# crate-crypto/rust-eth-kzg

Measured on AMD Instinct MI355X. Metric: blobs/sec compute_cells_and_kzg_proofs (4096-pt blob), higher is better.
Workload: dtype u32

## Files before the change

### rust-eth-kzg_amd/csrc/engine.hip

```cpp
#include "engine_internal.hpp"

namespace kzg {

static Fr fr_from_u64(uint64_t v) {
    Fr a = zero<FrParams>();
    a.v[0] = (uint32_t)v;
    a.v[1] = (uint32_t)(v >> 32);
    return to_mont(a);
}
static Fr fr_pow_limbs(const Fr& base, const uint32_t* e, int nl) {
    Fr acc = one<FrParams>();
    for (int i = 32 * nl - 1; i >= 0; i--) {
        acc = sqr(acc);
        if ((e[i >> 5] >> (i & 31)) & 1) acc = mul(acc, base);
    }
    return acc;
}
static Fr fr_root_of_unity(int log_n) {
    uint32_t e[8];
    for (int i = 0; i < 8; i++) e[i] = FrParams::MOD[i];
    e[0] -= 1;
    for (int s = 0; s < log_n; s++) {
        for (int i = 0; i < 8; i++) e[i] = (e[i] >> 1) | (i < 7 ? (e[i + 1] << 31) : 0);
    }
    return fr_pow_limbs(fr_from_u64(7), e, 8);
}
typedef unsigned __int128 u128;
static const u128 GLV_LAMBDA = ((u128)0xac45a4010001a402ULL << 64) | 0x00000000ffffffffULL;
static void glv_split(const Fr& canon, u128& k1, u128& k2) {
    u128 rem = 0, q = 0;
    for (int i = 255; i >= 0; i--) {
        bool top = (rem >> 127) & 1;
        rem = (rem << 1) | ((canon.v[i >> 5] >> (i & 31)) & 1);
        q <<= 1;
        if (top || rem >= GLV_LAMBDA) { rem -= GLV_LAMBDA; q |= 1; }
    }
    k1 = rem;
    k2 = q;
}
static void recode_glv_wnaf(const Fr& k_mont, const Fr& lambda_mont, uint32_t* out) {
    constexpr int TWW = launch::TWIDDLE_WORDS, W = launch::TWIDDLE_WNAF_W;
    u128 r, q;
    glv_split(from_mont(k_mont), r, q);
    struct Half { u128 mag; bool neg; };
    auto signed_sub = [](u128 a, u128 b) { return a >= b ? Half{a - b, false} : Half{b - a, true}; };
    const Half cand[4][2] = {
        {Half{r, false}, Half{q, false}},
        {signed_sub(r, GLV_LAMBDA), Half{q + 1, false}},
        {signed_sub(r, 1), signed_sub(q, GLV_LAMBDA + 1)},
        {signed_sub(r, GLV_LAMBDA + 1), signed_sub(q, GLV_LAMBDA)},
    };
    auto fr_of = [](const Half& h) {
        Fr a = zero<FrParams>();
        for (int i = 0; i < 4; i++) a.v[i] = (uint32_t)(h.mag >> (32 * i));
        a = to_mont(a);
        return h.neg ? neg(a) : a;
    };
    auto naf = [&](const Half& h, int8_t* dg, int& len, int& weight) {
        u128 v = h.mag;
        len = weight = 0;
        for (int t = 0; v != 0; t++, v >>= 1) {
            if (t >= 4 * TWW) throw std::runtime_error("constant recoding too long");
            if (!(v & 1)) continue;
            int d = (int)(v & ((1u << W) - 1));
            if (d >= (1 << (W - 1))) d -= 1 << W;
            if (d < 0) v += (u128)(-d); else v -= (u128)d;
            dg[t] = (int8_t)(h.neg ? -d : d);
            len = t + 1;
            weight++;
        }
    };
    double best_cost = 0;
    int best = -1;
    std::vector<uint32_t> best_words;
    for (int c = 0; c < 4; c++) {
        if (!eq(add(fr_of(cand[c][0]), mul(fr_of(cand[c][1]), lambda_mont)), k_mont)) throw std::runtime_error("GLV split failed");
        std::vector<uint32_t> words(2 * TWW, 0u);
        int len[2], wt[2];
        for (int h = 0; h < 2; h++) naf(cand[c][h], reinterpret_cast<int8_t*>(&words[(size_t)h * TWW]), len[h], wt[h]);
        const double cost = linmap::COST_DBL * std::max(len[0], len[1]) + 5.0e3 * (wt[0] + wt[1]);
        if (best < 0 || cost < best_cost) { best = c; best_cost = cost; best_words = words; }
    }
    for (int i = 0; i < 2 * TWW; i++) out[i] = best_words[i];
    for (int h = 0; h < 2; h++) {
        const int8_t* dg = reinterpret_cast<const int8_t*>(out + (size_t)h * TWW);
        Fr back = zero<FrParams>(), pw = one<FrParams>();
        for (int t = 0; t < 4 * TWW; t++, pw = add(pw, pw)) {
            const int d = dg[t];
            if (!d) continue;
            Fr term = pw;
            for (int m = 1; m < (d < 0 ? -d : d); m++) term = add(term, pw);
            back = d < 0 ? sub(back, term) : add(back, term);
        }
        if (!eq(back, fr_of(cand[best][h]))) throw std::runtime_error("constant recoding failed");
    }
}
double trace_clock_ms() {
    static const auto t0 = std::chrono::steady_clock::now();
    return std::chrono::duration<double, std::milli>(std::chrono::steady_clock::now() - t0).count();
}
static thread_local std::string t_last_error;
const std::string& Engine::last_error() const { return t_last_error; }
void Engine::set_error(const std::exception& e) { t_last_error = e.what(); }

BufferPool::~BufferPool() {
    for (auto& f : free_) {
        if (host_) (void)hipHostFree(f.second);
        else (void)hipFree(f.second);
    }
}
void* BufferPool::get(size_t bytes, size_t* cls) {
    size_t c = 256;
    while (c < bytes) c <<= 1;
    *cls = c;
    for (size_t i = 0; i < free_.size(); i++)
        if (free_[i].first == c) {
            void* p = free_[i].second;
            free_[i] = free_.back();
            free_.pop_back();
            pooled_ -= c;
            return p;
        }
    void* p = nullptr;
    hipError_t e = host_ ? hipHostMalloc(&p, c, hipHostMallocDefault) : hipMalloc(&p, c);
    if (e != hipSuccess) {
        (void)hipGetLastError();
        for (auto& f : free_) { if (host_) (void)hipHostFree(f.second); else (void)hipFree(f.second); }
        free_.clear();
        pooled_ = 0;
        e = host_ ? hipHostMalloc(&p, c, hipHostMallocDefault) : hipMalloc(&p, c);
        if (e != hipSuccess) throw std::runtime_error(host_ ? "hipHostMalloc failed" : "hipMalloc failed");
    }
    return p;
}
void BufferPool::put(void* p, size_t cls) {
    constexpr size_t KEEP = 6ull << 30;
    if (pooled_ + cls > KEEP) {
        if (host_) (void)hipHostFree(p); else (void)hipFree(p);
        return;
    }
    free_.emplace_back(cls, p);
    pooled_ += cls;
}
PoolBuf::PoolBuf(Engine& e, size_t bytes, bool pinned_host) : e_(e), host_(pinned_host) {
    p = (host_ ? e_.pin_pool_ : e_.dev_pool_).get(bytes ? bytes : 1, &cls_);
}
PoolBuf::~PoolBuf() {
    (void)hipStreamSynchronize(e_.stream_);
    (host_ ? e_.pin_pool_ : e_.dev_pool_).put(p, cls_);
}

std::atomic<bool> g_exiting{false};
std::mutex g_engines_mu;
std::vector<Engine*> g_engines;
void Engine::stop_builder() {
    cancel_build_.store(true);
    if (builder_.joinable()) builder_.join();
}
void stop_all_builders_at_exit() {
    g_exiting.store(true);
    std::vector<Engine*> live;
    {
        std::lock_guard<std::mutex> lk(g_engines_mu);
        live = g_engines;
    }
    for (Engine* e : live) e->stop_builder();
}

Engine::SerialLease Engine::lease_serial() {
    return lanes_.lease(this, max_lanes_, auxiliary_, [this] {
        try {
            return std::unique_ptr<Engine>(new Engine(use_precomp_, dev_, this));
        } catch (...) {
            (void)hipGetLastError();
            throw;
        }
    });
}

Engine::Engine(bool use_precomp, int device, const Engine* primary, double table_budget_gb) : dev_(device), use_precomp_(use_precomp), primary_(primary), auxiliary_(primary != nullptr) {
    knobs_ = primary ? primary->knobs_ : Knobs::from_env();
    if (knobs_.serial_lanes) max_lanes_ = knobs_.serial_lanes;
    if (knobs_.device_batch_max) device_batch_max_ = ((knobs_.device_batch_max + 63) / 64) * 64;
    if (use_precomp) {
        if (launch::glv_width_supported(knobs_.glv_window)) want_glv_c_ = knobs_.glv_window;
        if (table_budget_gb != 0) table_budget_gb_ = table_budget_gb;
        else if (knobs_.table_budget_gb != 0) table_budget_gb_ = knobs_.table_budget_gb;
    }
    vm_search_ = knobs_.vm_search;
    arena_signed_ = knobs_.arena_signed;
    msm_split_ = knobs_.msm_split;
    if (knobs_.pip_shift_min >= 1) pip_shift_min_ = knobs_.pip_shift_min;
#ifdef KZG_CIRC_MAX
    circ_max_ = KZG_CIRC_MAX;
#else
    circ_max_ = 2;
#endif
    try {
        construct();
    } catch (...) {
        teardown();
        throw;
    }
}

void Engine::construct() {
    const bool trace = knobs_.trace;
    auto t0 = std::chrono::steady_clock::now();
    auto lap = [&](const char* what) {
        if (!trace) return;
        auto t1 = std::chrono::steady_clock::now();
        fprintf(stderr, "[context] %-28s %8.1f ms\n", what, std::chrono::duration<double, std::milli>(t1 - t0).count());
        t0 = t1;
    };
    HIPCK(hipSetDevice(dev_));
    {
        int cus = 0;
        HIPCK(hipDeviceGetAttribute(&cus, hipDeviceAttributeMultiprocessorCount, dev_));
        wave_slots_ = cus * 4 * 2;
        if (knobs_.msm_chunks >= 0) msm_chunks_ = knobs_.msm_chunks;
    }
    HIPCK(hipStreamCreateWithFlags(&stream_, hipStreamNonBlocking));
    if (!primary_) {
        int prio_low = 0, prio_high = 0;
        HIPCK(hipDeviceGetStreamPriorityRange(&prio_low, &prio_high));
        HIPCK(hipStreamCreateWithPriority(&build_stream_, hipStreamNonBlocking, prio_low));
    }
    if (v_two_streams_) HIPCK(hipStreamCreateWithFlags(&v_side_, hipStreamNonBlocking));
    HIPCK(hipEventCreateWithFlags(&v_decoded_, hipEventDisableTiming));
    HIPCK(hipEventCreateWithFlags(&v_checked_, hipEventDisableTiming));
    for (Work& w : work_) {
        HIPCK(hipEventCreateWithFlags(&w.done, hipEventDisableTiming));
        HIPCK(hipEventCreateWithFlags(&w.ev_in, hipEventDisableTiming));
        HIPCK(hipEventCreateWithFlags(&w.ev_cells, hipEventDisableTiming));
        HIPCK(hipEventCreateWithFlags(&w.ev_cells_host, hipEventDisableTiming));
        HIPCK(hipEventCreateWithFlags(&w.ev_done, hipEventDisableTiming));
        HIPCK(hipEventCreateWithFlags(&w.ev_coeffs, hipEventDisableTiming));
        HIPCK(hipEventCreateWithFlags(&w.ev_side, hipEventDisableTiming));
        if (&w == &work_[0]) continue;
        if (primary_) continue;
        int prio_low = 0, prio_high = 0;
        HIPCK(hipDeviceGetStreamPriorityRange(&prio_low, &prio_high));
        HIPCK(hipStreamCreateWithFlags(&w.stream, hipStreamNonBlocking));
        HIPCK(hipStreamCreateWithPriority(&w.copy, hipStreamNonBlocking, prio_high));
    }
    launch::init_attributes();
    if (!primary_) settle_streams();
    lap("HIP runtime + stream");
    init_constants();
    lap("twiddles, recodings");
    init_srs();
    lap("SRS decompress");
    init_fk20();
    lap("FK20 bases + start tables");
    init_verifier();
    HIPCK(hipStreamSynchronize(stream_));
    lap("verifier (G2 lines, cosets)");
    if (knobs_.fault == "constructor" && !primary_) throw std::runtime_error("injected fault (ETH_KZG_AMD_FAULT=constructor)");
    start_builder();
}

bool Engine::streams_overlap(hipStream_t a, hipStream_t b) {
    int khz = 0;
    if (hipDeviceGetAttribute(&khz, hipDeviceAttributeWallClockRate, dev_) != hipSuccess || khz <= 0) khz = 100000;
    const double spin_us = 300.0;
    const uint64_t ticks = (uint64_t)(spin_us * 1e-3 * khz);
    for (int t = 0; t < 3; t++) {
        HIPCK(hipStreamSynchronize(a));
        HIPCK(hipStreamSynchronize(b));
        const auto t0 = std::chrono::steady_clock::now();
        launch::spin(ticks, a);
        launch::spin(ticks, b);
        HIPCK(hipStreamSynchronize(a));
        HIPCK(hipStreamSynchronize(b));
        const double us = std::chrono::duration<double, std::micro>(std::chrono::steady_clock::now() - t0).count();
        if (us < 1.6 * spin_us) return true;
    }
    return false;
}
void Engine::settle_streams() {
    const bool trace = knobs_.trace;
    launch::spin(1, stream_);
    std::vector<hipStream_t> chosen{stream_}, rejected;
    bool gave_up = false;
    for (int i = 1; i < NW; i++) {
        Work& w = work_[i];
        if (!w.stream || gave_up) continue;
        for (int attempt = 0;; attempt++) {
            launch::spin(1, w.stream);
            bool ok = true;
            for (hipStream_t c : chosen) ok = ok && streams_overlap(c, w.stream);
            if (ok || attempt == 5) {
                if (trace) fprintf(stderr, "[eth_kzg_amd] work set %d: stream %s after %d replacement(s)\n", i, ok ? "runs beside the others" : "still shares a queue", attempt);
                if (!ok) gave_up = true;
                break;
            }
            rejected.push_back(w.stream);
            HIPCK(hipStreamCreateWithFlags(&w.stream, hipStreamNonBlocking));
        }
        chosen.push_back(w.stream);
    }
    for (hipStream_t r : rejected) hipStreamDestroy(r);
}

Engine::~Engine() { teardown(); }

void Engine::teardown() noexcept {
    (void)hipSetDevice(dev_);
    lanes_.clear();
    stop_builder();
    {
        std::lock_guard<std::mutex> lk(g_engines_mu);
        g_engines.erase(std::remove(g_engines.begin(), g_engines.end(), this), g_engines.end());
    }
    if (build_stream_) hipStreamDestroy(build_stream_);
    host_pool_.reset();
    vm_pool_.reset();
    stage_pool_.reset();
    void* ptrs[] = {d_w8192_, d_w29_, d_naf_, d_srs_, d_fk_bases_, d_in_, d_cells_, d_proofs_, d_coset_, d_coset_inv_, d_circ_terms_};
    for (void* p : ptrs)
        if (p) hipFree(p);
    for (SlpProgram& P : slp_prog_) {
        if (P.d_words) hipFree(P.d_words);
        if (P.d_naf && P.owns_naf) hipFree(P.d_naf);
    }
    for (Work& w : work_) {
        void* dev[] = {w.coeffs, w.canon, w.scalars, w.X, w.status, w.circ_table, w.slp_arena, w.d_in, w.d_cells, w.d_proofs};
        for (void* p : dev)
            if (p) hipFree(p);
        void* pin[] = {w.h_in, w.h_cells, w.h_proofs, w.h_status};
        for (void* p : pin)
            if (p) hipHostFree(p);
        hipEvent_t evs[] = {w.done, w.ev_in, w.ev_cells, w.ev_cells_host, w.ev_done, w.ev_coeffs, w.ev_side};
        for (hipEvent_t e : evs)
            if (e) hipEventDestroy(e);
        for (hipEvent_t e : w.sub_events) hipEventDestroy(e);
        if (w.stream) hipStreamDestroy(w.stream);
        if (w.copy) hipStreamDestroy(w.copy);
    }
    if (v_dev_) hipFree(v_dev_);
    if (v_pin_) hipHostFree(v_pin_);
    for (VmSlot& v : vm_slot_) {
        if (v.dev) hipFree(v.dev);
        if (v.pin) hipHostFree(v.pin);
        if (v.vs.dev) hipFree(v.vs.dev);
        if (v.vs.pin) hipHostFree(v.vs.pin);
    }
    if (vd_pin_) hipHostFree(vd_pin_);
    for (hipEvent_t e : vd_events_)
        if (e) hipEventDestroy(e);
    if (v_side_) hipStreamDestroy(v_side_);
    if (v_decoded_) hipEventDestroy(v_decoded_);
    if (v_checked_) hipEventDestroy(v_checked_);
    if (stream_) hipStreamDestroy(stream_);
}

void Engine::init_constants() {
    std::vector<Fr> w(N_EXT);
    Fr g = fr_root_of_unity(13);
    w[0] = one<FrParams>();
    for (int i = 1; i < N_EXT; i++) w[i] = mul(w[i - 1], g);
    if (!eq(mul(w[N_EXT - 1], g), one<FrParams>())) throw std::runtime_error("omega_8192 has wrong order");
    HIPCK(hipMalloc(&d_w8192_, N_EXT * sizeof(Fr)));
    HIPCK(hipMemcpy(d_w8192_, w.data(), N_EXT * sizeof(Fr), hipMemcpyHostToDevice));
    {
        std::vector<uint32_t> w29((size_t)N_EXT * 9);
        launch::ntt_twiddles29(w.data(), w29.data());
        HIPCK(hipMalloc(&d_w29_, w29.size() * 4));
        HIPCK(hipMemcpy(d_w29_, w29.data(), w29.size() * 4, hipMemcpyHostToDevice));
    }
    {
        Fr lam = zero<FrParams>();
        for (int i = 0; i < 4; i++) lam.v[i] = (uint32_t)(GLV_LAMBDA >> (32 * i));
        Fr lm = to_mont(lam);
        if (!is_zero(add(add(sqr(lm), lm), one<FrParams>()))) throw std::runtime_error("GLV lambda is not a cube root of unity");
        constexpr int TWW = launch::TWIDDLE_WORDS;
        std::vector<uint32_t> tw((size_t)128 * 2 * TWW, 0u);
        for (int k = 0; k < 128; k++) recode_glv_wnaf(w[64 * k], lm, &tw[(size_t)k * 2 * TWW]);
        HIPCK(hipMalloc(&d_naf_, tw.size() * 4));
        HIPCK(hipMemcpy(d_naf_, tw.data(), tw.size() * 4, hipMemcpyHostToDevice));
        std::vector<uint32_t> plus, minus;
        int max_t = 0;
        for (int d = 0; d < 128; d++) {
            Fr c = zero<FrParams>();
            for (int t = 0; t < 64; t++) c = add(c, w[(64 * d * t) & (N_EXT - 1)]);
            if (d != 0 && (d & 1) == 0) {
                if (!is_zero(c)) throw std::runtime_error("circulant symbol: even entry is not zero");
                continue;
            }
            u128 kk[2];
            glv_split(from_mont(c), kk[0], kk[1]);
            Fr back = zero<FrParams>();
            for (int half = 0; half < 2; half++) {
                u128 k = kk[half];
                Fr pw = half ? lm : one<FrParams>();
                for (int t = 0; k != 0; t++, k >>= 1, pw = add(pw, pw)) {
                    if (!(k & 1)) continue;
                    const int dg = 2 - (int)(k & 3);
                    if (dg < 0) k += 1;
                    const uint32_t word = (uint32_t)d | ((uint32_t)t << 7) | ((uint32_t)half << 15) | ((dg < 0 ? 1u : 0u) << 16) | (1u << 17);
                    (dg < 0 ? minus : plus).push_back(word);
                    back = dg < 0 ? sub(back, pw) : add(back, pw);
                    if (t > max_t) max_t = t;
                }
            }
            if (!eq(back, c)) throw std::runtime_error("circulant term list does not reproduce its symbol");
        }
        if ((int)plus.size() < launch::CIRC_LANES || max_t >= 255) throw std::runtime_error("circulant term list is malformed");
        std::vector<uint32_t> all(plus);
        all.insert(all.end(), minus.begin(), minus.end());
        circ_T_ = max_t + 1;
        circ_per_lane_ = ((int)all.size() + launch::CIRC_LANES - 1) / launch::CIRC_LANES;
        all.resize((size_t)circ_per_lane_ * launch::CIRC_LANES, 0u);
        HIPCK(hipMalloc(&d_circ_terms_, all.size() * 4));
        HIPCK(hipMemcpy(d_circ_terms_, all.data(), all.size() * 4, hipMemcpyHostToDevice));
    }
    init_linmap(reinterpret_cast<const Fr8*>(w.data()));
    for (int sgi = 0; sgi < 3; sgi++) {
        Fr v = zero<FrParams>();
        v.v[sgi + 1] = 1;
        v = to_mont(v);
        memcpy(&seg_shift_[sgi], &v, 32);
    }
    Fr i4096 = inv(fr_from_u64(N_BLOB)), i128 = inv(fr_from_u64(128));
    memcpy(&n_inv4096_, &i4096, 32);
    memcpy(&inv128_, &i128, 32);
}

static linmap::Strategy slp_strategy(int id) {
    linmap::Strategy s;
    s.allow_toom8 = true;
    auto fixed = [&](int k4, int k8, int k16, int k32) {
        s.tuned = false;
        s.balanced_lincomb = true;
        s.hankel_split = {{2, 2}, {4, k4}, {8, k8}, {16, k16}, {32, k32}};
    };
    switch (id) {
        case 2: fixed(2, 2, 2, 2); break;
        case 3: fixed(4, 2, 4, 2); break;
        case 4: fixed(2, 2, 2, 4); break;
        case 5: fixed(4, 2, 4, 8); break;
        default: break;
    }
    return s;
}
void Engine::build_slp_program(int id) {
    const Fr* w128p = reinterpret_cast<const Fr*>(w128_.data());
    const std::vector<Fr> w128(w128p, w128p + 128);
    const bool verbose = knobs_.trace;
    linmap::Plan plan = linmap::build_fk20_proofs_plan(w128, slp_strategy(id), verbose);
    {
        std::vector<linmap::Ref> perm(128);
        for (int p = 0; p < 128; p++) {
            int k = 0;
            for (int b = 0; b < 7; b++) k |= ((p >> b) & 1) << (6 - b);
            perm[p] = plan.outputs[k];
        }
        plan.outputs = perm;
    }
    const linmap::Schedule sched = linmap::make_schedule(plan, id == SLP_TUNED_FUSED);
    uint64_t st = 0x853c49e6748fea9bull + (uint64_t)id;
    for (int it = 0; it < 2; it++) {
        std::vector<Fr> in(128);
        for (auto& v : in) {
            for (int i = 0; i < 8; i++) { st ^= st << 13; st ^= st >> 7; st ^= st << 17; v.v[i] = (uint32_t)(st >> 16); }
            v.v[7] &= 0x3fffffffu;
        }
        const auto want = linmap::fk20_proofs_map_by_definition(w128, in);
        const auto got1 = linmap::run_over_fr(plan, in);
        const auto got2 = linmap::run_schedule_over_fr(sched, plan.consts, 128, 128, in);
        for (int p = 0; p < 128; p++) {
            int k = 0;
            for (int b = 0; b < 7; b++) k |= ((p >> b) & 1) << (6 - b);
            if (!eq(want[k], got1[p]) || !eq(want[k], got2[p])) throw std::runtime_error("FK20 proofs map: compiled program differs from its definition");
        }
    }
    SlpProgram& P = slp_prog_[id];
    if (id == SLP_TUNED && slp_prog_[SLP_TUNED_FUSED].ready) {
        P.d_naf = slp_prog_[SLP_TUNED_FUSED].d_naf;
    } else {
        Fr lam = zero<FrParams>();
        for (int i = 0; i < 4; i++) lam.v[i] = (uint32_t)(GLV_LAMBDA >> (32 * i));
        const Fr lm = to_mont(lam);
        constexpr int TWW = launch::TWIDDLE_WORDS;
        std::vector<uint32_t> naf(plan.consts.size() * 2 * TWW);
        for (size_t c = 0; c < plan.consts.size(); c++) recode_glv_wnaf(plan.consts[c], lm, &naf[c * 2 * TWW]);
        HIPCK(hipMalloc(&P.d_naf, naf.size() * 4));
        P.owns_naf = true;
        HIPCK(hipMemcpy(P.d_naf, naf.data(), naf.size() * 4, hipMemcpyHostToDevice));
    }
    HIPCK(hipMalloc(&P.d_words, sched.words.size() * 4));
    HIPCK(hipMemcpy(P.d_words, sched.words.data(), sched.words.size() * 4, hipMemcpyHostToDevice));
    P.launches.clear();
    for (auto& L : sched.launches) P.launches.push_back(SlpLaunch{(int)L.kind, L.first, L.count});
    P.n_slots = sched.n_slots;
    P.info[0] = (int)plan.count(linmap::OP_MULC);
    P.info[1] = (int)(plan.count(linmap::OP_ADD) + plan.count(linmap::OP_SUB));
    P.info[2] = (int)plan.doublings();
    P.info[3] = (int)sched.launches.size();
    if (verbose) fprintf(stderr, "[linmap] program %d: %d multiplications, %d additions, %d doublings, %d launches, %d slots\n", id, P.info[0], P.info[1], P.info[2], P.info[3], P.n_slots);
    P.ready = true;
}
const Engine::SlpProgram& Engine::slp_program(int id) {
    std::lock_guard<std::mutex> lk(slp_build_mu_);
    if (!slp_prog_[id].ready) build_slp_program(id);
    return slp_prog_[id];
}
int Engine::pick_slp_program(int lanes) const {
    if (slp_force_ >= 0) return slp_force_;
    const int groups = lanes / 64, simds = wave_slots_ / 2;
    if (712 * groups <= simds) return SLP_KARATSUBA;
    if (456 * groups <= simds) return SLP_DEPTH_456;
    if (606 * groups <= wave_slots_) return SLP_DEPTH_606;
    if (456 * groups <= wave_slots_) return SLP_DEPTH_456;
    if (372 * groups <= wave_slots_) return SLP_DEPTH_372;
    if (456 * groups <= wave_slots_ * 3 / 2) return SLP_DEPTH_456;
    if (groups <= 12) return SLP_DEPTH_372;
    return lanes >= slp_fuse_min_ ? SLP_TUNED_FUSED : SLP_TUNED;
}
void Engine::init_linmap(const Fr8* w8192_mont) {
    static_assert(sizeof(Fr8) == sizeof(Fr), "layout");
    if (knobs_.slp_program >= 0 && knobs_.slp_program < SLP_COUNT) slp_force_ = knobs_.slp_program;
    w128_.resize(128);
    for (int e = 0; e < 128; e++) w128_[e] = w8192_mont[64 * e];
    build_slp_program(SLP_TUNED_FUSED);
    build_slp_program(SLP_TUNED);
    const SlpProgram& fused = slp_prog_[SLP_TUNED_FUSED];
    {
        if (fused.info[0] != slp_prog_[SLP_TUNED].info[0]) throw std::runtime_error("FK20 proofs map: the two schedules differ");
    }
    for (int i = 0; i < 3; i++) slp_info_[i] = fused.info[i];
    slp_info_[3] = fused.info[3];
    const Fr h = inv(fr_from_u64(2));
    memcpy(&half_, &h, 32);
}

void Engine::init_srs() {
    const unsigned char* p = kzg_srs_begin;
    size_t len = (size_t)(kzg_srs_end - kzg_srs_begin);
    uint32_t n1, n2;
    if (len < 16 || memcmp(p, "KZGSRS01", 8)) throw std::runtime_error("bad embedded SRS");
    memcpy(&n1, p + 8, 4);
    memcpy(&n2, p + 12, 4);
    if (n1 != (uint32_t)N_BLOB || len != 16 + (size_t)n1 * 48 + (size_t)n2 * 96) throw std::runtime_error("bad embedded SRS size");
    uint8_t* d_bytes;
    int* d_st;
    HIPCK(hipMalloc(&d_bytes, (size_t)N_BLOB * 48));
    HIPCK(hipMalloc(&d_st, N_BLOB * sizeof(int)));
    HIPCK(hipMalloc(&d_srs_, N_BLOB * sizeof(G1Affine)));
    HIPCK(hipMemcpy(d_bytes, p + 16, (size_t)N_BLOB * 48, hipMemcpyHostToDevice));
    {
        Fp12w nobeta{};
        launch::g1_decompress(d_bytes, d_srs_, d_st, N_BLOB, 0, nobeta, stream_);
    }
    std::vector<int> st(N_BLOB);
    HIPCK(hipMemcpyAsync(st.data(), d_st, N_BLOB * sizeof(int), hipMemcpyDeviceToHost, stream_));
    HIPCK(hipStreamSynchronize(stream_));
    for (int s : st)
        if (s) throw std::runtime_error("embedded SRS point failed to decompress");
    HIPCK(hipFree(d_bytes));
    HIPCK(hipFree(d_st));
    {
        G1Affine P;
        HIPCK(hipMemcpy(&P, (const G1Affine*)d_srs_ + 1, sizeof(G1Affine), hipMemcpyDeviceToHost));
        uint32_t lam[4];
        for (int i = 0; i < 4; i++) lam[i] = (uint32_t)(GLV_LAMBDA >> (32 * i));
        G1Affine Q = to_affine(scalar_mul<4>(to_jac(P), lam));
        Fp bx = mul(Q.x, inv(P.x));
        Fp b3 = mul(sqr(bx), bx);
        if (!eq(b3, one<FpParams>()) || eq(bx, one<FpParams>()) || !eq(Q.y, P.y)) throw std::runtime_error("GLV endomorphism check failed");
        memcpy(&beta_, &bx, 48);
    }
}

}
```

### rust-eth-kzg_amd/csrc/g1_linmap.hpp

```cpp
#pragma once
#include "field.hpp"

#include <algorithm>
#include <cstdint>
#include <cstdio>
#include <functional>
#include <map>
#include <stdexcept>
#include <tuple>
#include <vector>

namespace kzg {
namespace linmap {

enum OpKind : uint8_t { OP_ADD = 0, OP_SUB = 1, OP_DBL = 2, OP_MULC = 3 };
struct Op {
    OpKind kind;
    int dst;
    int a;
    int b;
};
struct Ref {
    int id = -1;
    bool neg = false;
    bool zero() const { return id < 0; }
};

struct Plan {
    int n_in = 0;
    int n_values = 0;
    std::vector<Op> ops;
    std::vector<Ref> outputs;
    std::vector<Fr> consts;
    long count(OpKind k) const {
        long n = 0;
        for (auto& o : ops) n += o.kind == k;
        return n;
    }
    long doublings() const {
        long n = 0;
        for (auto& o : ops) n += o.kind == OP_DBL ? o.b : 0;
        return n;
    }
};

constexpr double COST_MULC = 690e3, COST_ADD = 8.3e3, COST_DBL = 3.1e3;

inline Fr fr_small(int64_t v) {
    Fr a = zero<FrParams>();
    uint64_t m = v < 0 ? (uint64_t)(-v) : (uint64_t)v;
    a.v[0] = (uint32_t)m;
    a.v[1] = (uint32_t)(m >> 32);
    a = to_mont(a);
    return v < 0 ? neg(a) : a;
}

class Builder {
public:
    explicit Builder(int n_in) {
        plan_.n_in = n_in;
        plan_.n_values = n_in;
    }
    Ref input(int i) const { return Ref{i, false}; }
    static Ref negate(Ref r) { return r.zero() ? r : Ref{r.id, !r.neg}; }

    Ref add(Ref a, Ref b) {
        if (a.zero()) return b;
        if (b.zero()) return a;
        if (a.id == b.id) return a.neg == b.neg ? dbl(a, 1) : Ref{};
        if (!a.neg && !b.neg) return Ref{emit2(OP_ADD, a.id, b.id, true), false};
        if (a.neg && b.neg) return Ref{emit2(OP_ADD, a.id, b.id, true), true};
        if (!a.neg) return Ref{emit2(OP_SUB, a.id, b.id, false), false};
        return Ref{emit2(OP_SUB, b.id, a.id, false), false};
    }
    Ref sub(Ref a, Ref b) { return add(a, negate(b)); }
    Ref dbl(Ref a, int t) {
        if (a.zero() || t == 0) return a;
        auto key = std::make_tuple((int)OP_DBL, a.id, t);
        auto it = memo_.find(key);
        if (it != memo_.end()) return Ref{it->second, a.neg};
        int id = plan_.n_values++;
        plan_.ops.push_back(Op{OP_DBL, id, a.id, t});
        memo_[key] = id;
        return Ref{id, a.neg};
    }
    Ref mulc(Ref a, const Fr& c) {
        if (a.zero() || is_zero(c)) return Ref{};
        if (eq(c, one<FrParams>())) return a;
        if (eq(c, neg(one<FrParams>()))) return negate(a);
        int cid = (int)plan_.consts.size();
        plan_.consts.push_back(c);
        int id = plan_.n_values++;
        plan_.ops.push_back(Op{OP_MULC, id, a.id, cid});
        return Ref{id, a.neg};
    }
    Ref lincomb(const std::vector<std::pair<Ref, int64_t>>& terms) {
        std::vector<std::pair<Ref, uint64_t>> t;
        int top = -1;
        for (auto& pr : terms) {
            if (pr.first.zero() || pr.second == 0) continue;
            Ref r = pr.second < 0 ? negate(pr.first) : pr.first;
            uint64_t m = pr.second < 0 ? (uint64_t)(-pr.second) : (uint64_t)pr.second;
            t.emplace_back(r, m);
            for (int b = 63; b >= 0; b--)
                if ((m >> b) & 1) { if (b > top) top = b; break; }
        }
        Ref acc;
        int pending = 0;
        for (int b = top; b >= 0; b--) {
            if (!acc.zero()) pending++;
            if (b == top) pending = 0;
            for (auto& pr : t)
                if ((pr.second >> b) & 1) {
                    if (pending) { acc = dbl(acc, pending); pending = 0; }
                    acc = add(acc, pr.first);
                }
        }
        if (pending) acc = dbl(acc, pending);
        return acc;
    }
    Ref lincomb_balanced(const std::vector<std::pair<Ref, int64_t>>& terms) {
        struct T { Ref r; int e; };
        std::vector<T> t;
        for (auto& pr : terms) {
            if (pr.first.zero() || pr.second == 0) continue;
            const uint64_t m = pr.second < 0 ? (uint64_t)(-pr.second) : (uint64_t)pr.second;
            if (m & (m - 1)) return lincomb(terms);
            int e = 0;
            while (!((m >> e) & 1)) e++;
            t.push_back(T{pr.second < 0 ? negate(pr.first) : pr.first, e});
        }
        if (t.empty()) return Ref{};
        std::stable_sort(t.begin(), t.end(), [](const T& a, const T& b) { return a.e < b.e; });
        std::function<Ref(int, int)> rec = [&](int lo, int hi) -> Ref {
            if (hi - lo == 1) return t[lo].r;
            const int mid = (lo + hi) / 2;
            const Ref a = rec(lo, mid), b = rec(mid, hi);
            return add(dbl(b, t[mid].e - t[lo].e), a);
        };
        return dbl(rec(0, (int)t.size()), t[0].e);
    }
    Plan take(const std::vector<Ref>& outputs) {
        plan_.outputs = outputs;
        return std::move(plan_);
    }
    const Plan& plan() const { return plan_; }
    double cost() const { return plan_.count(OP_MULC) * COST_MULC + (plan_.count(OP_ADD) + plan_.count(OP_SUB)) * COST_ADD + plan_.doublings() * COST_DBL; }

private:
    int emit2(OpKind k, int a, int b, bool commutative) {
        if (commutative && a > b) std::swap(a, b);
        auto key = std::make_tuple((int)k, a, b);
        auto it = memo_.find(key);
        if (it != memo_.end()) return it->second;
        int id = plan_.n_values++;
        plan_.ops.push_back(Op{k, id, a, b});
        memo_[key] = id;
        return id;
    }
    Plan plan_;
    std::map<std::tuple<int, int, int>, int> memo_;
};

struct EvalPoint { int a, b; };
inline std::vector<EvalPoint> toom_points(int k) {
    switch (k) {
        case 2: return {{0, 1}, {1, 0}, {1, 1}};
        case 3: return {{0, 1}, {1, 0}, {1, 1}, {-1, 1}, {2, 1}};
        case 4: return {{0, 1}, {1, 0}, {1, 1}, {-1, 1}, {2, 1}, {-2, 1}, {1, 2}};
        case 8: return {{0, 1}, {1, 0}, {1, 1}, {-1, 1}, {2, 1}, {-2, 1}, {1, 2}, {-1, 2}, {4, 1}, {-4, 1}, {1, 4}, {-1, 4}, {8, 1}, {-8, 1}, {1, 8}};
        default: throw std::runtime_error("toom_points: unsupported split");
    }
}
inline int64_t ipow(int64_t b, int e) {
    int64_t r = 1;
    while (e-- > 0) r *= b;
    return r;
}
inline std::vector<std::vector<Fr>> toom_fixed_side(int k) {
    const auto pts = toom_points(k);
    const int R = 2 * k - 1;
    std::vector<std::vector<Fr>> M(R, std::vector<Fr>(2 * R, zero<FrParams>()));
    for (int s = 0; s < R; s++) {
        for (int r = 0; r < R; r++) M[s][r] = fr_small(ipow(pts[r].a, s) * ipow(pts[r].b, 2 * k - 2 - s));
        M[s][R + s] = one<FrParams>();
    }
    for (int col = 0; col < R; col++) {
        int piv = -1;
        for (int row = col; row < R; row++)
            if (!is_zero(M[row][col])) { piv = row; break; }
        if (piv < 0) throw std::runtime_error("toom: singular evaluation matrix");
        std::swap(M[piv], M[col]);
        const Fr iv = inv(M[col][col]);
        for (int j = 0; j < 2 * R; j++) M[col][j] = mul(M[col][j], iv);
        for (int row = 0; row < R; row++) {
            if (row == col || is_zero(M[row][col])) continue;
            const Fr f = M[row][col];
            for (int j = 0; j < 2 * R; j++) M[row][j] = sub(M[row][j], mul(f, M[col][j]));
        }
    }
    std::vector<std::vector<Fr>> U(R, std::vector<Fr>(R));
    for (int r = 0; r < R; r++)
        for (int D = 0; D < R; D++) U[r][D] = M[r][R + D];
    return U;
}

class Compiler {
public:
    std::map<int, int> hankel_split;
    std::map<int, bool> root_split;
    bool allow_toom8 = true;
    bool balanced_lincomb = false;
    Ref sum(Builder& B, const std::vector<std::pair<Ref, int64_t>>& t) const { return balanced_lincomb ? B.lincomb_balanced(t) : B.lincomb(t); }

    std::vector<Ref> hankel(Builder& B, const std::vector<Ref>& x, const std::vector<Fr>& h) {
        const int n = (int)x.size();
        if ((int)h.size() != 2 * n - 1) throw std::runtime_error("hankel: size mismatch");
        if (n == 1) return {B.mulc(x[0], h[0])};
        const int k = hankel_split.count(n) ? hankel_split[n] : 2;
        if (n % k) throw std::runtime_error("hankel: split does not divide the size");
        const int m = n / k, R = 2 * k - 1;
        const auto pts = toom_points(k);
        const auto& U = fixed_side(k);
        std::vector<std::vector<Ref>> X(R, std::vector<Ref>(m));
        std::vector<int> partner(R, -1);
        for (int r = 0; r < R; r++)
            for (int q = 0; q < R; q++)
                if (q != r && pts[q].a == -pts[r].a && pts[q].b == pts[r].b && pts[r].a > 0) { partner[r] = q; partner[q] = r; }
        for (int r = 0; r < R; r++) {
            if (partner[r] >= 0 && pts[r].a < 0) continue;
            for (int i = 0; i < m; i++) {
                if (partner[r] < 0) {
                    std::vector<std::pair<Ref, int64_t>> t;
                    for (int J = 0; J < k; J++) t.emplace_back(x[J * m + i], ipow(pts[r].a, J) * ipow(pts[r].b, k - 1 - J));
                    X[r][i] = sum(B, t);
                } else {
                    std::vector<std::pair<Ref, int64_t>> ev, od;
                    for (int J = 0; J < k; J++) (J & 1 ? od : ev).emplace_back(x[J * m + i], ipow(pts[r].a, J) * ipow(pts[r].b, k - 1 - J));
                    const Ref e = sum(B, ev), o = sum(B, od);
                    X[r][i] = B.add(e, o);
                    X[partner[r]][i] = B.sub(e, o);
                }
            }
        }
        std::vector<std::vector<Ref>> Z(R);
        for (int r = 0; r < R; r++) {
            std::vector<Fr> hr(2 * m - 1, zero<FrParams>());
            for (int D = 0; D < R; D++) {
                if (is_zero(U[r][D])) continue;
                for (int s = 0; s < 2 * m - 1; s++) hr[s] = add(hr[s], mul(U[r][D], h[D * m + s]));
            }
            Z[r] = hankel(B, X[r], hr);
        }
        std::vector<Ref> y(n);
        for (int i = 0; i < m; i++) {
            std::vector<Ref> S(R), Dm(R);
            for (int r = 0; r < R; r++)
                if (partner[r] >= 0 && pts[r].a > 0) {
                    S[r] = B.add(Z[r][i], Z[partner[r]][i]);
                    Dm[r] = B.sub(Z[r][i], Z[partner[r]][i]);
                }
            for (int I = 0; I < k; I++) {
                std::vector<std::pair<Ref, int64_t>> t;
                for (int r = 0; r < R; r++) {
                    if (partner[r] >= 0 && pts[r].a < 0) continue;
                    const int64_t coef = ipow(pts[r].a, I) * ipow(pts[r].b, k - 1 - I);
                    if (partner[r] < 0) t.emplace_back(Z[r][i], coef);
                    else t.emplace_back((I & 1) ? Dm[r] : S[r], coef);
                }
                y[I * m + i] = sum(B, t);
            }
        }
        return y;
    }

    template <class SqrtFn>
    std::vector<Ref> twisted_cyclic(Builder& B, const std::vector<Ref>& x, const std::vector<Fr>& c, const Fr& z, SqrtFn&& sqrt_of) {
        const int n = (int)x.size();
        Fr s;
        if (n >= 2 && root_split.count(n) && root_split[n] && sqrt_of(z, s)) {
            const int hn = n / 2;
            const Fr half = inv(fr_small(2)), s_inv = inv(s);
            std::vector<Ref> x1(hn), x2(hn);
            std::vector<Fr> c1(hn), c2(hn);
            for (int i = 0; i < hn; i++) {
                const Ref t = B.mulc(x[hn + i], s);
                x1[i] = B.add(x[i], t);
                x2[i] = B.sub(x[i], t);
                const Fr sc = mul(s, c[hn + i]);
                c1[i] = mul(half, add(c[i], sc));
                c2[i] = mul(half, sub(c[i], sc));
            }
            const auto y1 = twisted_cyclic(B, x1, c1, s, sqrt_of);
            const auto y2 = twisted_cyclic(B, x2, c2, neg(s), sqrt_of);
            std::vector<Ref> y(n);
            for (int i = 0; i < hn; i++) {
                y[i] = B.add(y1[i], y2[i]);
                y[hn + i] = B.mulc(B.sub(y1[i], y2[i]), s_inv);
            }
            return y;
        }
        std::vector<Fr> h(2 * n - 1);
        for (int u = 0; u < 2 * n - 1; u++) {
            const int d = u - (n - 1);
            h[u] = d >= 0 ? c[d] : mul(z, c[n + d]);
        }
        std::vector<Ref> xr(n);
        for (int j = 0; j < n; j++) xr[j] = x[n - 1 - j];
        return hankel(B, xr, h);
    }

    template <class SqrtFn>
    std::vector<Ref> cyclic(Builder& B, const std::vector<Ref>& x, const std::vector<Fr>& c, SqrtFn&& sqrt_of) {
        const int n = (int)x.size();
        if (n == 1) return {B.mulc(x[0], c[0])};
        const int hn = n / 2;
        const Fr half = inv(fr_small(2));
        std::vector<Ref> xp(hn), xm(hn);
        std::vector<Fr> cp(hn), cm(hn);
        for (int i = 0; i < hn; i++) {
            xp[i] = B.add(x[i], x[hn + i]);
            xm[i] = B.sub(x[i], x[hn + i]);
            cp[i] = mul(half, add(c[i], c[hn + i]));
            cm[i] = mul(half, sub(c[i], c[hn + i]));
        }
        const auto yp = cyclic(B, xp, cp, sqrt_of);
        const auto ym = twisted_cyclic(B, xm, cm, neg(one<FrParams>()), sqrt_of);
        std::vector<Ref> y(n);
        for (int i = 0; i < hn; i++) {
            y[i] = B.add(yp[i], ym[i]);
            y[hn + i] = B.sub(yp[i], ym[i]);
        }
        return y;
    }

    void tune(int max_n) {
        uint64_t st = 0x9e3779b97f4a7c15ull;
        auto rnd_fr = [&]() {
            Fr a;
            for (int i = 0; i < 8; i++) { st ^= st << 13; st ^= st >> 7; st ^= st << 17; a.v[i] = (uint32_t)(st >> 16); }
            a.v[7] &= 0x3fffffffu;
            return a;
        };
        auto no_sqrt = [](const Fr&, Fr&) { return false; };
        auto any_sqrt = [&](const Fr&, Fr& s) { s = rnd_fr(); return true; };
        for (int n = 2; n <= max_n; n *= 2) {
            double best = 0;
            int best_k = 0;
            for (int k : {2, 4, 8}) {
                if (n % k || (k == 8 && !allow_toom8)) continue;
                hankel_split[n] = k;
                Builder B(n);
                std::vector<Ref> x(n);
                for (int i = 0; i < n; i++) x[i] = B.input(i);
                std::vector<Fr> h(2 * n - 1);
                for (auto& v : h) v = rnd_fr();
                hankel(B, x, h);
                if (!best_k || B.cost() < best) { best = B.cost(); best_k = k; }
            }
            hankel_split[n] = best_k;
            double cost[2];
            for (int split = 0; split < 2; split++) {
                root_split[n] = split != 0;
                Builder B(n);
                std::vector<Ref> x(n);
                for (int i = 0; i < n; i++) x[i] = B.input(i);
                std::vector<Fr> c(n);
                for (auto& v : c) v = rnd_fr();
                if (split) twisted_cyclic(B, x, c, rnd_fr(), any_sqrt);
                else twisted_cyclic(B, x, c, rnd_fr(), no_sqrt);
                cost[split] = B.cost();
            }
            root_split[n] = cost[1] < cost[0];
        }
    }

private:
    const std::vector<std::vector<Fr>>& fixed_side(int k) {
        auto it = fixed_.find(k);
        if (it == fixed_.end()) it = fixed_.emplace(k, toom_fixed_side(k)).first;
        return it->second;
    }
    std::map<int, std::vector<std::vector<Fr>>> fixed_;
};

inline std::vector<Fr> run_over_fr(const Plan& p, const std::vector<Fr>& in) {
    std::vector<Fr> v(p.n_values, zero<FrParams>());
    for (int i = 0; i < p.n_in; i++) v[i] = in[i];
    for (auto& o : p.ops) {
        switch (o.kind) {
            case OP_ADD: v[o.dst] = add(v[o.a], v[o.b]); break;
            case OP_SUB: v[o.dst] = sub(v[o.a], v[o.b]); break;
            case OP_DBL: { Fr t = v[o.a]; for (int k = 0; k < o.b; k++) t = add(t, t); v[o.dst] = t; break; }
            case OP_MULC: v[o.dst] = mul(v[o.a], p.consts[o.b]); break;
        }
    }
    std::vector<Fr> out(p.outputs.size());
    for (size_t i = 0; i < out.size(); i++) {
        const Ref r = p.outputs[i];
        out[i] = r.zero() ? zero<FrParams>() : (r.neg ? neg(v[r.id]) : v[r.id]);
    }
    return out;
}

struct Strategy {
    bool tuned = true, allow_toom8 = true;
    std::map<int, int> hankel_split;
    std::map<int, bool> root_split;
    bool balanced_lincomb = false;
};
inline Plan build_fk20_proofs_plan(const std::vector<Fr>& w128, const Strategy& strat, bool verbose = false) {
    if (w128.size() != 128) throw std::runtime_error("w128: need the 128 powers");
    auto sqrt_of = [&](const Fr& z, Fr& s) {
        for (int e = 0; e < 128; e += 2)
            if (eq(z, w128[e])) { s = w128[e / 2]; return true; }
        return false;
    };
    Compiler C;
    C.allow_toom8 = strat.allow_toom8;
    C.balanced_lincomb = strat.balanced_lincomb;
    if (strat.tuned) C.tune(32);
    else { C.hankel_split = strat.hankel_split; C.root_split = strat.root_split; }
    Builder B(128);
    const Fr one_ = one<FrParams>(), inv32 = inv(fr_small(32));
    auto m_of = [&](int e) {
        return mul(inv32, inv(sub(one_, w128[((e % 128) + 128) % 128])));
    };
    std::vector<Ref> even(64), odd(64);
    for (int a = 0; a < 64; a++) { even[a] = B.input(2 * a); odd[a] = B.input(2 * a + 1); }
    std::vector<Fr> c1(64), c2(64);
    for (int d = 0; d < 64; d++) { c1[d] = m_of(2 * d - 1); c2[d] = m_of(2 * d + 1); }
    const auto t1 = C.cyclic(B, odd, c1, sqrt_of);
    const auto t2 = C.cyclic(B, even, c2, sqrt_of);
    std::vector<Ref> out(128);
    for (int a = 0; a < 64; a++) {
        out[2 * a] = B.add(even[a], t1[a]);
        out[2 * a + 1] = B.add(odd[a], t2[a]);
    }
    for (auto& r : out)
        if (r.zero() || r.neg || r.id < 128) throw std::runtime_error("fk20 plan: degenerate output");
    Plan p = B.take(out);
    if (verbose) {
        fprintf(stderr, "[linmap] hankel splits:");
        for (auto& kv : C.hankel_split) fprintf(stderr, " %d->%d", kv.first, kv.second);
        fprintf(stderr, "  root splits:");
        for (auto& kv : C.root_split) fprintf(stderr, " %d:%d", kv.first, (int)kv.second);
        fprintf(stderr, "\n[linmap] %ld constant multiplications, %ld additions, %ld doublings\n", p.count(OP_MULC),
                p.count(OP_ADD) + p.count(OP_SUB), p.doublings());
    }
    return p;
}
inline Plan build_fk20_proofs_plan(const std::vector<Fr>& w128, bool allow_toom8 = true, bool verbose = false) {
    Strategy s;
    s.allow_toom8 = allow_toom8;
    return build_fk20_proofs_plan(w128, s, verbose);
}

inline std::vector<Fr> fk20_proofs_map_by_definition(const std::vector<Fr>& w128, const std::vector<Fr>& in) {
    const Fr inv64 = inv(fr_small(64));
    std::vector<Fr> h(64), out(128);
    for (int n = 0; n < 64; n++) {
        Fr acc = zero<FrParams>();
        for (int j = 0; j < 128; j++) acc = add(acc, mul(in[j], w128[(128 - (j * n) % 128) % 128]));
        h[n] = mul(acc, inv64);
    }
    for (int k = 0; k < 128; k++) {
        Fr acc = zero<FrParams>();
        for (int n = 0; n < 64; n++) acc = add(acc, mul(h[n], w128[(k * n) % 128]));
        out[k] = acc;
    }
    return out;
}

struct Launch {
    OpKind kind;
    int first, count;
};
struct Schedule {
    int n_slots = 0;
    std::vector<uint32_t> words;
    std::vector<Launch> launches;
    long mulc_total = 0;
    long fused_pairs = 0;
    long fused_runs = 0;
};
inline Schedule make_schedule(const Plan& p, bool fuse_add_sub = true, bool fuse_runs = true) {
    const int n_out = (int)p.outputs.size();
    std::vector<char> live(p.n_values, 0);
    for (auto& r : p.outputs) live[r.id] = 1;
    for (int i = (int)p.ops.size() - 1; i >= 0; i--) {
        const Op& o = p.ops[i];
        if (!live[o.dst]) continue;
        live[o.a] = 1;
        if (o.kind == OP_ADD || o.kind == OP_SUB) live[o.b] = 1;
    }
    std::vector<int> run_of(p.n_values, 0);
    std::vector<int> run_src(p.n_values, -1);
    if (fuse_runs) {
        std::vector<std::vector<int>> users(p.n_values);
        std::vector<char> is_output(p.n_values, 0);
        for (auto& r : p.outputs) is_output[r.id] = 1;
        for (int i = 0; i < (int)p.ops.size(); i++) {
            const Op& o = p.ops[i];
            if (!live[o.dst]) continue;
            users[o.a].push_back(i);
            if (o.kind == OP_ADD || o.kind == OP_SUB) users[o.b].push_back(i);
        }
        for (auto& o : p.ops) {
            if (!live[o.dst] || o.kind != OP_DBL || is_output[o.dst] || o.b > 31) continue;
            const auto& u = users[o.dst];
            auto two = [&](int k) { return p.ops[k].kind == OP_ADD || p.ops[k].kind == OP_SUB; };
            auto fits = [&](const Op& c) {
                const int other = c.a == o.dst ? c.b : c.a;
                return c.a != c.b && !run_of[other] && (c.kind == OP_ADD || c.a == o.dst);
            };
            bool ok = false;
            if (u.size() == 1 && two(u[0]) && fits(p.ops[u[0]])) ok = true;
            if (fuse_add_sub && u.size() == 2 && two(u[0]) && two(u[1]) && p.ops[u[0]].kind != p.ops[u[1]].kind) {
                const Op &x = p.ops[u[0]], &y = p.ops[u[1]];
                if (std::min(x.a, x.b) == std::min(y.a, y.b) && std::max(x.a, x.b) == std::max(y.a, y.b) && fits(x) && fits(y)) ok = true;
            }
            if (!ok) continue;
            run_of[o.dst] = o.b;
            run_src[o.dst] = o.a;
        }
    }
    auto eff = [&](int v) { return run_of[v] ? run_src[v] : v; };
    std::vector<int> md(p.n_values, 0), lvl(p.n_values, 0);
    int max_md = 0;
    std::vector<int> max_lvl;
    for (auto& o : p.ops) {
        if (!live[o.dst]) continue;
        const bool two = o.kind == OP_ADD || o.kind == OP_SUB;
        if (run_of[o.dst]) {
            md[o.dst] = md[o.a];
            lvl[o.dst] = lvl[o.a];
            continue;
        }
        if (o.kind == OP_MULC) {
            md[o.dst] = md[o.a] + 1;
            lvl[o.dst] = 0;
        } else {
            md[o.dst] = two ? std::max(md[o.a], md[o.b]) : md[o.a];
            int l = 0;
            if (md[o.a] == md[o.dst]) l = std::max(l, lvl[o.a] + 1);
            if (two && md[o.b] == md[o.dst]) l = std::max(l, lvl[o.b] + 1);
            lvl[o.dst] = std::max(l, 1);
        }
        max_md = std::max(max_md, md[o.dst]);
        if ((int)max_lvl.size() <= md[o.dst]) max_lvl.resize(md[o.dst] + 1, 0);
        max_lvl[md[o.dst]] = std::max(max_lvl[md[o.dst]], lvl[o.dst]);
    }
    std::vector<std::vector<int>> step_ops;
    std::map<std::pair<int, int>, int> step_of;
    for (int ph = 0; ph <= max_md; ph++)
        for (int l = 0; l <= (ph < (int)max_lvl.size() ? max_lvl[ph] : 0); l++) {
            step_of[{ph, l}] = (int)step_ops.size();
            step_ops.emplace_back();
        }
    std::vector<int> def_step(p.n_values, -1), last_use(p.n_values, -1);
    for (int i = 0; i < (int)p.ops.size(); i++) {
        const Op& o = p.ops[i];
        if (!live[o.dst] || run_of[o.dst]) continue;
        const int s = step_of[{md[o.dst], lvl[o.dst]}];
        step_ops[s].push_back(i);
        def_step[o.dst] = s;
        last_use[eff(o.a)] = std::max(last_use[eff(o.a)], s);
        if (o.kind == OP_ADD || o.kind == OP_SUB) last_use[eff(o.b)] = std::max(last_use[eff(o.b)], s);
    }
    Schedule S;
    std::vector<int> slot(p.n_values, -1);
    for (int i = 0; i < p.n_in; i++) slot[i] = i;
    for (int k = 0; k < n_out; k++) {
        if (slot[p.outputs[k].id] >= 0) throw std::runtime_error("schedule: an output value is shared or is an input");
        slot[p.outputs[k].id] = p.n_in + k;
    }
    int next_slot = p.n_in + n_out;
    std::vector<int> free_list;
    std::vector<std::vector<int>> expire(step_ops.size() + 1);
    for (int v = p.n_in; v < p.n_values; v++)
        if (live[v] && slot[v] < 0 && last_use[v] >= 0) expire[last_use[v]].push_back(v);
    for (int s = 0; s < (int)step_ops.size(); s++) {
        for (int i : step_ops[s]) {
            const int v = p.ops[i].dst;
            if (slot[v] >= 0) continue;
            if (!free_list.empty()) { slot[v] = free_list.back(); free_list.pop_back(); }
            else slot[v] = next_slot++;
        }
        for (int v : expire[s]) free_list.push_back(slot[v]);
        std::map<std::pair<int, int>, int> add_of;
        for (int i : step_ops[s])
            if (p.ops[i].kind == OP_ADD) add_of[{std::min(p.ops[i].a, p.ops[i].b), std::max(p.ops[i].a, p.ops[i].b)}] = i;
        std::map<int, int> partner;
        std::vector<char> fused_away(p.ops.size(), 0);
        if (fuse_add_sub)
            for (int i : step_ops[s]) {
                if (p.ops[i].kind != OP_SUB) continue;
                auto it = add_of.find({std::min(p.ops[i].a, p.ops[i].b), std::max(p.ops[i].a, p.ops[i].b)});
                if (it == add_of.end() || fused_away[it->second]) continue;
                partner[i] = it->second;
                fused_away[it->second] = 1;
            }
        std::vector<int> ordered = step_ops[s];
        auto op_cost = [&](int i) {
            const Op& o = p.ops[i];
            if (o.kind == OP_DBL) return o.b * COST_DBL;
            if (o.kind == OP_MULC) return COST_MULC;
            return (run_of[o.a] + run_of[o.b]) * COST_DBL + (partner.count(i) ? 1.15 * COST_ADD : COST_ADD);
        };
        std::stable_sort(ordered.begin(), ordered.end(), [&](int x, int y) { return op_cost(x) > op_cost(y); });
        for (int pass = 0; pass < 2; pass++) {
            Launch L{pass == 0 ? OP_MULC : OP_ADD, (int)S.words.size() / 4, 0};
            for (int i : ordered) {
                const Op& o = p.ops[i];
                const bool two = o.kind == OP_ADD || o.kind == OP_SUB;
                if ((pass == 0) != (o.kind == OP_MULC)) continue;
                if (fused_away[i]) continue;
                int first = o.a, second = two ? o.b : 0;
                if (two && run_of[o.b]) std::swap(first, second);
                const uint32_t shifts = two ? (uint32_t)run_of[first] << 3 : 0u;
                if (two && run_of[first]) S.fused_runs++;
                if (partner.count(i)) {
                    S.words.push_back((uint32_t)slot[p.ops[partner[i]].dst]);
                    S.words.push_back((uint32_t)slot[eff(first)]);
                    S.words.push_back((uint32_t)slot[eff(second)]);
                    S.words.push_back(4u | shifts | ((uint32_t)slot[o.dst] << 16));
                    L.count++;
                    S.fused_pairs++;
                    continue;
                }
                S.words.push_back((uint32_t)slot[o.dst]);
                S.words.push_back((uint32_t)slot[two ? eff(first) : o.a]);
                S.words.push_back(two ? (uint32_t)slot[eff(second)] : (uint32_t)o.b);
                S.words.push_back((o.kind == OP_SUB ? 1u : o.kind == OP_DBL ? 2u : 0u) | shifts);
                L.count++;
            }
            if (L.count) S.launches.push_back(L);
            if (pass == 0) S.mulc_total += L.count;
        }
    }
    S.n_slots = next_slot;
    return S;
}

inline std::vector<Fr> run_schedule_over_fr(const Schedule& S, const std::vector<Fr>& consts, int n_in, int n_out, const std::vector<Fr>& in) {
    std::vector<Fr> arena(S.n_slots, zero<FrParams>());
    for (int i = 0; i < n_in; i++) arena[i] = in[i];
    for (auto& L : S.launches) {
        std::vector<Fr> res(L.count), res2(L.count);
        for (int i = 0; i < L.count; i++) {
            const uint32_t* w = &S.words[(size_t)(L.first + i) * 4];
            const Fr a = arena[w[1]];
            if (L.kind == OP_MULC) res[i] = mul(a, consts[w[2]]);
            else if (w[3] & 2u) { Fr t = a; for (uint32_t k = 0; k < w[2]; k++) t = add(t, t); res[i] = t; }
            else {
                Fr x = a, y = arena[w[2]];
                for (uint32_t k = 0; k < ((w[3] >> 3) & 31u); k++) x = add(x, x);
                if (w[3] & 4u) { res[i] = add(x, y); res2[i] = sub(x, y); }
                else res[i] = (w[3] & 1u) ? sub(x, y) : add(x, y);
            }
        }
        for (int i = 0; i < L.count; i++) {
            const uint32_t* w = &S.words[(size_t)(L.first + i) * 4];
            arena[w[0]] = res[i];
            if (L.kind != OP_MULC && (w[3] & 4u)) arena[w[3] >> 16] = res2[i];
        }
    }
    return std::vector<Fr>(arena.begin() + n_in, arena.begin() + n_in + n_out);
}

}
}
```

### rust-eth-kzg_amd/csrc/k_g1slp.hip

```cpp
#include "engine.hpp"
#include <stdexcept>
#include "g1_mulc.hpp"
#include "g1_mulc30.hpp"
#include "g1_coop.hpp"

namespace kzg {

static_assert(sizeof(JacS) == launch::SIZEOF_JACS && sizeof(JacQ) == launch::SIZEOF_JACQ, "the engine sizes and offsets the arena with these");

__global__ __launch_bounds__(64, 2) void k_slp_mulc(JacQ* __restrict__ A, int stride, const uint32_t* __restrict__ words,
                                                    const uint32_t* __restrict__ naf, Fs<1, DC> beta, int n_active) {
    const uint32_t* w = words + (size_t)blockIdx.x * 4;
    const uint32_t dst = __builtin_amdgcn_readfirstlane(w[0]), a = __builtin_amdgcn_readfirstlane(w[1]),
                   cid = __builtin_amdgcn_readfirstlane(w[2]);
    const int lane = (gridDim.y - 1 - blockIdx.y) * 64 + threadIdx.x;
    if (lane >= n_active) return;
    const JacQ src = A[(size_t)a * stride + lane];
    A[(size_t)dst * stride + lane] = mul_by_recoded30(src, naf + (size_t)cid * (2 * launch::TWIDDLE_WORDS), beta);
}
__global__ __launch_bounds__(64, 2) void k_slp_mulc_s(JacS* __restrict__ A, int stride, const uint32_t* __restrict__ words,
                                                      const uint32_t* __restrict__ naf, Fs<1, DC> beta, int n_active) {
    const uint32_t* w = words + (size_t)blockIdx.x * 4;
    const uint32_t dst = __builtin_amdgcn_readfirstlane(w[0]), a = __builtin_amdgcn_readfirstlane(w[1]),
                   cid = __builtin_amdgcn_readfirstlane(w[2]);
    const int lane = (gridDim.y - 1 - blockIdx.y) * 64 + threadIdx.x;
    const JacS src = A[(size_t)a * stride + (lane < n_active ? lane : n_active - 1)];
    const JacS r = mul_by_recoded30(src, naf + (size_t)cid * (2 * launch::TWIDDLE_WORDS), beta);
    if (lane < n_active) A[(size_t)dst * stride + lane] = r;
}
__global__ __launch_bounds__(64, 2) void k_slp_mulc_coop(JacQ* __restrict__ A, int stride, const uint32_t* __restrict__ words,
                                                         const uint32_t* __restrict__ naf, Fq<1> beta, int lanes) {
    const uint32_t* w = words + (size_t)blockIdx.x * 4;
    const uint32_t dst = __builtin_amdgcn_readfirstlane(w[0]), a = __builtin_amdgcn_readfirstlane(w[1]),
                   cid = __builtin_amdgcn_readfirstlane(w[2]);
    const int lane = blockIdx.y * 16 + (threadIdx.x >> 2), quad = threadIdx.x & 3;
    if (lane >= lanes) return;
    const JacQ src = A[(size_t)a * stride + lane];
    A[(size_t)dst * stride + lane] = mul_by_recoded<4>(src, naf + (size_t)cid * (2 * launch::TWIDDLE_WORDS), beta, quad);
}
__global__ __launch_bounds__(64, 2) void k_slp_mulc_coop2(JacQ* __restrict__ A, int stride, const uint32_t* __restrict__ words,
                                                          const uint32_t* __restrict__ naf, Fq<1> beta, int lanes) {
    const uint32_t* w = words + (size_t)blockIdx.x * 4;
    const uint32_t dst = __builtin_amdgcn_readfirstlane(w[0]), a = __builtin_amdgcn_readfirstlane(w[1]),
                   cid = __builtin_amdgcn_readfirstlane(w[2]);
    const int lane = blockIdx.y * 32 + (threadIdx.x >> 1), half = threadIdx.x & 1;
    if (lane >= lanes) return;
    const JacQ src = A[(size_t)a * stride + lane];
    A[(size_t)dst * stride + lane] = mul_by_recoded<2>(src, naf + (size_t)cid * (2 * launch::TWIDDLE_WORDS), beta, half);
}
__device__ __forceinline__ void slp_cheap_op(JacQ* __restrict__ A, int stride, int lane, uint32_t dst, uint32_t a, uint32_t b, uint32_t fl) {
    JacQ r = A[(size_t)a * stride + lane];
    const uint32_t runs = (fl & 2u) ? b : (fl >> 3) & 31u;
#pragma unroll 1
    for (uint32_t k = 0; k < runs; k++) r = dbl(r);
    bool degenerate = false;
    if (!(fl & 2u)) {
        if (fl & 4u) {
            const AddSubShared sh = add_sub_prepare(r, A[(size_t)b * stride + lane]);
            degenerate = sh.degenerate;
            A[(size_t)(fl >> 16) * stride + lane] = add_sub_finish(sh, true);
            r = add_sub_finish(sh, false);
        } else {
            r = add(r, A[(size_t)b * stride + lane], (fl & 1u) != 0);
        }
    }
    A[(size_t)dst * stride + lane] = r;
    if (degenerate) {
        asm volatile("" ::: "memory");
        JacQ p2 = A[(size_t)a * stride + lane];
#pragma unroll 1
        for (uint32_t k = 0; k < runs; k++) p2 = dbl(p2);
        const JacQ q2 = A[(size_t)b * stride + lane];
        const JacQ d = add_slow(p2, q2, true);
        A[(size_t)dst * stride + lane] = add_slow(p2, q2, false);
        A[(size_t)(fl >> 16) * stride + lane] = d;
    }
}
__global__ __launch_bounds__(64, 2) void k_slp_add(JacQ* __restrict__ A, int stride, const uint32_t* __restrict__ words, int n_active) {
    const uint32_t* w = words + (size_t)blockIdx.y * 4;
    const uint32_t dst = __builtin_amdgcn_readfirstlane(w[0]), a = __builtin_amdgcn_readfirstlane(w[1]),
                   b = __builtin_amdgcn_readfirstlane(w[2]), fl = __builtin_amdgcn_readfirstlane(w[3]);
    if ((int)(blockIdx.x * 64 + threadIdx.x) >= n_active) return;
    slp_cheap_op(A, stride, blockIdx.x * 64 + threadIdx.x, dst, a, b, fl);
}

__global__ __launch_bounds__(64, 2) void k_slp_add_s(JacS* __restrict__ A, int stride, const uint32_t* __restrict__ words, int n_active) {
    const uint32_t* w = words + (size_t)blockIdx.y * 4;
    const uint32_t dst = __builtin_amdgcn_readfirstlane(w[0]), a = __builtin_amdgcn_readfirstlane(w[1]),
                   b = __builtin_amdgcn_readfirstlane(w[2]), fl = __builtin_amdgcn_readfirstlane(w[3]);
    const int lane_of_thread = blockIdx.x * 64 + threadIdx.x;
    const bool keep = lane_of_thread < n_active;
    const int lane = keep ? lane_of_thread : n_active - 1;
    JacS r = A[(size_t)a * stride + lane];
    const uint32_t runs = (fl & 2u) ? b : (fl >> 3) & 31u;
#pragma unroll 1
    for (uint32_t k = 0; k < runs; k++) r = dbl_half(r);
    bool degenerate = false;
    if (!(fl & 2u)) {
        if (fl & 4u) {
            const AddSubSharedS sh = add_sub_prepare(r, A[(size_t)b * stride + lane]);
            degenerate = sh.degenerate;
            const JacS df = add_sub_finish(sh, true);
            if (keep) A[(size_t)(fl >> 16) * stride + lane] = df;
            r = add_sub_finish(sh, false);
        } else {
            r = add_unchecked(r, A[(size_t)b * stride + lane], (fl & 1u) != 0, degenerate);
        }
    }
    if (keep) A[(size_t)dst * stride + lane] = r;
    if (degenerate && keep) {
        asm volatile("" ::: "memory");
        JacS p2 = A[(size_t)a * stride + lane];
#pragma unroll 1
        for (uint32_t k = 0; k < runs; k++) p2 = dbl_half(p2);
        const JacS q2 = A[(size_t)b * stride + lane];
        if (fl & 4u) {
            const JacS d = add_slow(p2, q2, true);
            A[(size_t)dst * stride + lane] = add_slow(p2, q2, false);
            A[(size_t)(fl >> 16) * stride + lane] = d;
        } else {
            A[(size_t)dst * stride + lane] = add_slow(p2, q2, (fl & 1u) != 0);
        }
    }
}

__global__ __launch_bounds__(64, 2) void k_slp_add_coop(JacQ* __restrict__ A, int stride, const uint32_t* __restrict__ words, int lanes) {
    const uint32_t* w = words + (size_t)blockIdx.y * 4;
    const uint32_t dst = __builtin_amdgcn_readfirstlane(w[0]), a = __builtin_amdgcn_readfirstlane(w[1]),
                   b = __builtin_amdgcn_readfirstlane(w[2]), fl = __builtin_amdgcn_readfirstlane(w[3]);
    const int lane = blockIdx.x * 16 + (threadIdx.x >> 2), quad = threadIdx.x & 3;
    if (lane >= lanes) return;
    JacQ r = A[(size_t)a * stride + lane];
    const uint32_t runs = (fl & 2u) ? b : (fl >> 3) & 31u;
#pragma unroll 1
    for (uint32_t k = 0; k < runs; k++) r = coop_dbl(r, quad);
    if (!(fl & 2u)) {
        const JacQ q = A[(size_t)b * stride + lane];
        if (fl & 4u) {
            const JacQ d = coop_add(r, q, true, quad);
            A[(size_t)(fl >> 16) * stride + lane] = d;
            r = coop_add(r, q, false, quad);
        } else {
            r = coop_add(r, q, (fl & 1u) != 0, quad);
        }
    }
    A[(size_t)dst * stride + lane] = r;
}

template <int COOP>
__global__ __launch_bounds__(64, 2) void k_slp_mulc_coop_s(JacS* __restrict__ A, int stride, const uint32_t* __restrict__ words,
                                                           const uint32_t* __restrict__ naf, Fs<1, DC> beta, int lanes) {
    const uint32_t* w = words + (size_t)blockIdx.x * 4;
    const uint32_t dst = __builtin_amdgcn_readfirstlane(w[0]), a = __builtin_amdgcn_readfirstlane(w[1]),
                   cid = __builtin_amdgcn_readfirstlane(w[2]);
    const int lane_of_thread = blockIdx.y * (64 / COOP) + (threadIdx.x / COOP), sub = threadIdx.x % COOP;
    const bool keep = lane_of_thread < lanes;
    const int lane = keep ? lane_of_thread : lanes - 1;
    const JacS src = A[(size_t)a * stride + lane];
    const JacS r = mul_by_recoded30<COOP>(src, naf + (size_t)cid * (2 * launch::TWIDDLE_WORDS), beta, sub);
    if (keep) A[(size_t)dst * stride + lane] = r;
}
__global__ __launch_bounds__(64, 2) void k_slp_add_coop_s(JacS* __restrict__ A, int stride, const uint32_t* __restrict__ words, int lanes) {
    const uint32_t* w = words + (size_t)blockIdx.y * 4;
    const uint32_t dst = __builtin_amdgcn_readfirstlane(w[0]), a = __builtin_amdgcn_readfirstlane(w[1]),
                   b = __builtin_amdgcn_readfirstlane(w[2]), fl = __builtin_amdgcn_readfirstlane(w[3]);
    const int lane_of_thread = blockIdx.x * 16 + (threadIdx.x >> 2), quad = threadIdx.x & 3;
    const bool keep = lane_of_thread < lanes;
    const int lane = keep ? lane_of_thread : lanes - 1;
    JacS r = A[(size_t)a * stride + lane];
    const uint32_t runs = (fl & 2u) ? b : (fl >> 3) & 31u;
#pragma unroll 1
    for (uint32_t k = 0; k < runs; k++) r = coop4_dbl_half(r, quad);
    if (!(fl & 2u)) {
        const JacS q = A[(size_t)b * stride + lane];
        if (fl & 4u) {
            JacS d;
            coop4_add_sub(r, q, quad, r, d);
            if (keep) A[(size_t)(fl >> 16) * stride + lane] = d;
        } else {
            r = coop4_add(r, q, (fl & 1u) != 0, quad);
        }
    }
    if (keep) A[(size_t)dst * stride + lane] = r;
}

namespace launch {
void preload_k_g1slp() {
    hipFuncAttributes a;
    (void)hipFuncGetAttributes(&a, reinterpret_cast<const void*>(&k_slp_add));
}
void g1_slp_launch(int kind, void* arena, int stride, const uint32_t* words, int count, const void* naf, const Fp12w& beta,
                   hipStream_t st, int lanes, int coop_lanes, int fmt, int n_active) {
    if (lanes <= 0) lanes = stride;
    if (n_active <= 0 || n_active > lanes) n_active = lanes;
    const dim3 grid((unsigned)count, (unsigned)(lanes / 64));
    if (fmt == FMT_JACS) {
        const bool coop = coop_points_max() > 0;
        if (kind == 3) {
            Fp b384;
            for (int i = 0; i < 12; i++) b384.v[i] = beta.v[i];
            const Fs<1, DC> bs = fs_from_fp(b384);
            if (coop_lanes > 16 && coop)
                k_slp_mulc_coop_s<2><<<dim3((unsigned)count, (unsigned)((coop_lanes + 31) / 32)), 64, 0, st>>>((JacS*)arena, stride, words, (const uint32_t*)naf, bs, coop_lanes);
            else if (coop_lanes > 0 && coop)
                k_slp_mulc_coop_s<4><<<dim3((unsigned)count, (unsigned)((coop_lanes + 15) / 16)), 64, 0, st>>>((JacS*)arena, stride, words, (const uint32_t*)naf, bs, coop_lanes);
            else k_slp_mulc_s<<<grid, 64, 0, st>>>((JacS*)arena, stride, words, (const uint32_t*)naf, bs, n_active);
        } else {
            if (lanes == 64 && count * 4 <= 1024 && coop)
                k_slp_add_coop_s<<<dim3((unsigned)((n_active + 15) / 16), (unsigned)count), 64, 0, st>>>((JacS*)arena, stride, words, n_active);
            else k_slp_add_s<<<dim3((unsigned)(lanes / 64), (unsigned)count), 64, 0, st>>>((JacS*)arena, stride, words, n_active);
        }
        return;
    }
    if (kind == 3) {
        Fp b384;
        for (int i = 0; i < 12; i++) b384.v[i] = beta.v[i];
        if (coop_lanes > 16 && coop_points_max() > 0) {
            const dim3 g2((unsigned)count, (unsigned)((coop_lanes + 31) / 32));
            k_slp_mulc_coop2<<<g2, 64, 0, st>>>((JacQ*)arena, stride, words, (const uint32_t*)naf, fq_from_fp(b384), coop_lanes);
        }
        else if (coop_lanes > 0 && coop_points_max() > 0)
            k_slp_mulc_coop<<<dim3((unsigned)count, (unsigned)((coop_lanes + 15) / 16)), 64, 0, st>>>((JacQ*)arena, stride, words, (const uint32_t*)naf,
                                                                                                     fq_from_fp(b384), coop_lanes);
        else k_slp_mulc<<<grid, 64, 0, st>>>((JacQ*)arena, stride, words, (const uint32_t*)naf, fs_from_fp(b384), n_active);
    } else {
        if (lanes == 64 && count * 4 <= 1024 && coop_points_max() > 0)
            k_slp_add_coop<<<dim3((unsigned)((n_active + 15) / 16), (unsigned)count), 64, 0, st>>>((JacQ*)arena, stride, words, n_active);
        else k_slp_add<<<dim3((unsigned)(lanes / 64), (unsigned)count), 64, 0, st>>>((JacQ*)arena, stride, words, n_active);
    }
}
}
}
```

Before: 40230.

## Use GLV endomorphism rotations as free Toom evaluation points in G1 linear-map SLP

Extends the straight-line program builder so references can carry a cube-root-of-unity rotation, applied on the GPU as the cheap G1 endomorphism (x multiplied by beta). Toom-Cook Hankel splits may then use evaluation points times powers of lambda and ±1 (the mu6 class scheme), which allows larger splits such as 16 and fewer scalar-multiplication (MULC) ops in the FK20 proof linear map. The add kernels now take beta and rotate their operands according to flag bits, and the cost model constants are retuned. The risks are extra per-add field multiplications and more complex plans, and the fixed strategies turn phi off.

```diff
diff --git a/rust-eth-kzg_amd/csrc/engine.hip b/rust-eth-kzg_amd/csrc/engine.hip
--- a/rust-eth-kzg_amd/csrc/engine.hip
+++ b/rust-eth-kzg_amd/csrc/engine.hip
@@ -430,9 +430,15 @@
 static linmap::Strategy slp_strategy(int id) {
     linmap::Strategy s;
     s.allow_toom8 = true;
+    {
+        Fr lam = zero<FrParams>();
+        for (int i = 0; i < 4; i++) lam.v[i] = (uint32_t)(GLV_LAMBDA >> (32 * i));
+        s.lambda = to_mont(lam);
+    }
     auto fixed = [&](int k4, int k8, int k16, int k32) {
         s.tuned = false;
         s.balanced_lincomb = true;
+        s.phi = false;
         s.hankel_split = {{2, 2}, {4, k4}, {8, k8}, {16, k16}, {32, k32}};
     };
     switch (id) {
diff --git a/rust-eth-kzg_amd/csrc/g1_linmap.hpp b/rust-eth-kzg_amd/csrc/g1_linmap.hpp
--- a/rust-eth-kzg_amd/csrc/g1_linmap.hpp
+++ b/rust-eth-kzg_amd/csrc/g1_linmap.hpp
@@ -19,12 +19,25 @@
     int dst;
     int a;
     int b;
+    int rot = 0;
 };
 struct Ref {
     int id = -1;
     bool neg = false;
+    int rot = 0;
     bool zero() const { return id < 0; }
 };
+
+inline Fr glv_lambda() {
+    static const uint32_t w[8] = {0xffffffffu, 0x00000000u, 0x0001a402u, 0xac45a401u, 0, 0, 0, 0};
+    Fr a = zero<FrParams>();
+    for (int i = 0; i < 8; i++) a.v[i] = w[i];
+    return to_mont(a);
+}
+inline Fr lambda_pow(const Fr& lambda, int rot) {
+    rot = ((rot % 3) + 3) % 3;
+    return rot == 0 ? one<FrParams>() : rot == 1 ? lambda : sqr(lambda);
+}
 
 struct Plan {
     int n_in = 0;
@@ -32,6 +45,7 @@
     std::vector<Op> ops;
     std::vector<Ref> outputs;
     std::vector<Fr> consts;
+    Fr lambda = glv_lambda();
     long count(OpKind k) const {
         long n = 0;
         for (auto& o : ops) n += o.kind == k;
@@ -42,9 +56,14 @@
         for (auto& o : ops) n += o.kind == OP_DBL ? o.b : 0;
         return n;
     }
+    long rotations() const {
+        long n = 0;
+        for (auto& o : ops) n += (o.kind == OP_ADD || o.kind == OP_SUB) && o.rot != 0;
+        return n;
+    }
 };
 
-constexpr double COST_MULC = 690e3, COST_ADD = 8.3e3, COST_DBL = 3.1e3;
+constexpr double COST_MULC = 564e3, COST_ADD = 7.0e3, COST_DBL = 2.8e3, COST_PHI = 0.48e3;
 
 inline Fr fr_small(int64_t v) {
     Fr a = zero<FrParams>();
@@ -57,42 +76,48 @@
 
 class Builder {
 public:
-    explicit Builder(int n_in) {
+    explicit Builder(int n_in, const Fr& lambda = glv_lambda()) {
         plan_.n_in = n_in;
         plan_.n_values = n_in;
-    }
-    Ref input(int i) const { return Ref{i, false}; }
-    static Ref negate(Ref r) { return r.zero() ? r : Ref{r.id, !r.neg}; }
+        plan_.lambda = lambda;
+    }
+    Ref input(int i) const { return Ref{i, false, 0}; }
+    static Ref negate(Ref r) { return r.zero() ? r : Ref{r.id, !r.neg, r.rot}; }
+    static Ref rotate(Ref r, int t) { return r.zero() ? r : Ref{r.id, r.neg, (((r.rot + t) % 3) + 3) % 3}; }
 
     Ref add(Ref a, Ref b) {
         if (a.zero()) return b;
         if (b.zero()) return a;
-        if (a.id == b.id) return a.neg == b.neg ? dbl(a, 1) : Ref{};
-        if (!a.neg && !b.neg) return Ref{emit2(OP_ADD, a.id, b.id, true), false};
-        if (a.neg && b.neg) return Ref{emit2(OP_ADD, a.id, b.id, true), true};
-        if (!a.neg) return Ref{emit2(OP_SUB, a.id, b.id, false), false};
-        return Ref{emit2(OP_SUB, b.id, a.id, false), false};
+        if (a.id == b.id) {
+            if (a.rot == b.rot) return a.neg == b.neg ? dbl(a, 1) : Ref{};
+            if (a.neg == b.neg) return Ref{a.id, !a.neg, 3 - a.rot - b.rot};
+        }
+        if (a.neg && !b.neg) std::swap(a, b);
+        const int r = (b.rot - a.rot + 3) % 3;
+        if (a.neg == b.neg) return Ref{emit2(OP_ADD, a.id, b.id, true, r), a.neg, a.rot};
+        return Ref{emit2(OP_SUB, a.id, b.id, false, r), false, a.rot};
     }
     Ref sub(Ref a, Ref b) { return add(a, negate(b)); }
     Ref dbl(Ref a, int t) {
         if (a.zero() || t == 0) return a;
-        auto key = std::make_tuple((int)OP_DBL, a.id, t);
+        auto key = std::make_tuple((int)OP_DBL, a.id, t, 0);
         auto it = memo_.find(key);
-        if (it != memo_.end()) return Ref{it->second, a.neg};
+        if (it != memo_.end()) return Ref{it->second, a.neg, a.rot};
         int id = plan_.n_values++;
         plan_.ops.push_back(Op{OP_DBL, id, a.id, t});
         memo_[key] = id;
-        return Ref{id, a.neg};
-    }
-    Ref mulc(Ref a, const Fr& c) {
+        return Ref{id, a.neg, a.rot};
+    }
+    Ref mulc(Ref a, Fr c) {
         if (a.zero() || is_zero(c)) return Ref{};
-        if (eq(c, one<FrParams>())) return a;
-        if (eq(c, neg(one<FrParams>()))) return negate(a);
+        c = mul(c, lambda_pow(plan_.lambda, a.rot));
+        if (eq(c, one<FrParams>())) return Ref{a.id, a.neg, 0};
+        if (eq(c, neg(one<FrParams>()))) return Ref{a.id, !a.neg, 0};
         int cid = (int)plan_.consts.size();
         plan_.consts.push_back(c);
         int id = plan_.n_values++;
         plan_.ops.push_back(Op{OP_MULC, id, a.id, cid});
-        return Ref{id, a.neg};
+        return Ref{id, a.neg, 0};
     }
     Ref lincomb(const std::vector<std::pair<Ref, int64_t>>& terms) {
         std::vector<std::pair<Ref, uint64_t>> t;
@@ -145,24 +170,31 @@
         return std::move(plan_);
     }
     const Plan& plan() const { return plan_; }
-    double cost() const { return plan_.count(OP_MULC) * COST_MULC + (plan_.count(OP_ADD) + plan_.count(OP_SUB)) * COST_ADD + plan_.doublings() * COST_DBL; }
+    double cost() const { return plan_cost(plan_); }
+    static double plan_cost(const Plan& p) {
+        return p.count(OP_MULC) * COST_MULC + (p.count(OP_ADD) + p.count(OP_SUB)) * COST_ADD + p.doublings() * COST_DBL + p.rotations() * COST_PHI;
+    }
 
 private:
-    int emit2(OpKind k, int a, int b, bool commutative) {
-        if (commutative && a > b) std::swap(a, b);
-        auto key = std::make_tuple((int)k, a, b);
+    int emit2(OpKind k, int a, int b, bool commutative, int rot) {
+        if (commutative && rot == 0 && a > b) std::swap(a, b);
+        auto key = std::make_tuple((int)k, a, b, rot);
         auto it = memo_.find(key);
         if (it != memo_.end()) return it->second;
         int id = plan_.n_values++;
-        plan_.ops.push_back(Op{k, id, a, b});
+        plan_.ops.push_back(Op{k, id, a, b, rot});
         memo_[key] = id;
         return id;
     }
     Plan plan_;
-    std::map<std::tuple<int, int, int>, int> memo_;
+    std::map<std::tuple<int, int, int, int>, int> memo_;
 };
 
-struct EvalPoint { int a, b; };
+struct EvalPoint {
+    int a, b;
+    int zr = 0;
+    bool zneg = false;
+};
 inline std::vector<EvalPoint> toom_points(int k) {
     switch (k) {
         case 2: return {{0, 1}, {1, 0}, {1, 1}};
@@ -172,17 +204,33 @@
         default: throw std::runtime_error("toom_points: unsupported split");
     }
 }
+inline std::vector<EvalPoint> toom_points_phi(int k) {
+    if (k == 2) return toom_points(2);
+    const int R = 2 * k - 1;
+    std::vector<EvalPoint> p = {{0, 1}, {1, 0}};
+    const int cls[][2] = {{1, 1}, {2, 1}, {1, 2}, {4, 1}, {1, 4}};
+    for (auto& c : cls)
+        for (int zr = 0; zr < 3; zr++)
+            for (int zn = 0; zn < 2; zn++)
+                if ((int)p.size() < R) p.push_back(EvalPoint{c[0], c[1], zr, zn != 0});
+    if ((int)p.size() != R) throw std::runtime_error("toom_points_phi: unsupported split");
+    return p;
+}
 inline int64_t ipow(int64_t b, int e) {
     int64_t r = 1;
     while (e-- > 0) r *= b;
     return r;
 }
-inline std::vector<std::vector<Fr>> toom_fixed_side(int k) {
-    const auto pts = toom_points(k);
+inline Fr point_coef(const EvalPoint& p, int J, int deg, const Fr& lambda) {
+    Fr c = mul(fr_small(ipow(p.a, J) * ipow(p.b, deg - J)), lambda_pow(lambda, p.zr * J));
+    return (p.zneg && (J & 1)) ? neg(c) : c;
+}
+inline std::vector<std::vector<Fr>> toom_fixed_side(int k, bool phi = false, const Fr& lambda = glv_lambda()) {
+    const auto pts = phi ? toom_points_phi(k) : toom_points(k);
     const int R = 2 * k - 1;
     std::vector<std::vector<Fr>> M(R, std::vector<Fr>(2 * R, zero<FrParams>()));
     for (int s = 0; s < R; s++) {
-        for (int r = 0; r < R; r++) M[s][r] = fr_small(ipow(pts[r].a, s) * ipow(pts[r].b, 2 * k - 2 - s));
+        for (int r = 0; r < R; r++) M[s][r] = point_coef(pts[r], s, 2 * k - 2, lambda);
         M[s][R + s] = one<FrParams>();
     }
     for (int col = 0; col < R; col++) {
@@ -211,6 +259,8 @@
     std::map<int, bool> root_split;
     bool allow_toom8 = true;
     bool balanced_lincomb = false;
+    bool phi = false;
+    Fr lambda = glv_lambda();
     Ref sum(Builder& B, const std::vector<std::pair<Ref, int64_t>>& t) const { return balanced_lincomb ? B.lincomb_balanced(t) : B.lincomb(t); }
 
     std::vector<Ref> hankel(Builder& B, const std::vector<Ref>& x, const std::vector<Fr>& h) {
@@ -219,6 +269,7 @@
         if (n == 1) return {B.mulc(x[0], h[0])};
         const int k = hankel_split.count(n) ? hankel_split[n] : 2;
         if (n % k) throw std::runtime_error("hankel: split does not divide the size");
+        if (phi && k > 2) return hankel_mu6(B, x, h, k);
         const int m = n / k, R = 2 * k - 1;
         const auto pts = toom_points(k);
         const auto& U = fixed_side(k);
@@ -274,6 +325,77 @@
         return y;
     }
 
+    std::vector<Ref> hankel_mu6(Builder& B, const std::vector<Ref>& x, const std::vector<Fr>& h, int k) {
+        const int n = (int)x.size(), m = n / k, R = 2 * k - 1;
+        const auto pts = toom_points_phi(k);
+        const auto& U = fixed_side(k);
+        struct Cls {
+            int a, b;
+            int member[3][2];
+        };
+        std::vector<Cls> cls;
+        for (int r = 0; r < R; r++) {
+            size_t c = 0;
+            while (c < cls.size() && !(cls[c].a == pts[r].a && cls[c].b == pts[r].b)) c++;
+            if (c == cls.size()) {
+                Cls nc{pts[r].a, pts[r].b, {{-1, -1}, {-1, -1}, {-1, -1}}};
+                cls.push_back(nc);
+            }
+            cls[c].member[pts[r].zr][pts[r].zneg ? 1 : 0] = r;
+        }
+        auto cf = [&](const Cls& c, int J) { return ipow(c.a, J) * ipow(c.b, k - 1 - J); };
+        std::vector<std::vector<Ref>> X(R, std::vector<Ref>(m));
+        for (auto& c : cls)
+            for (int i = 0; i < m; i++) {
+                Ref A[6];
+                for (int s = 0; s < 6 && s < k; s++) {
+                    std::vector<std::pair<Ref, int64_t>> t;
+                    for (int J = s; J < k; J += 6) t.emplace_back(x[J * m + i], cf(c, J));
+                    A[s] = sum(B, t);
+                }
+                for (int q = 0; q < 3; q++) {
+                    if (c.member[q][0] < 0 && c.member[q][1] < 0) continue;
+                    const Ref E = B.add(B.add(A[0], B.rotate(A[2], 2 * q)), B.rotate(A[4], q));
+                    const Ref O = B.add(B.add(B.rotate(A[1], q), A[3]), B.rotate(A[5], 2 * q));
+                    if (c.member[q][0] >= 0) X[c.member[q][0]][i] = B.add(E, O);
+                    if (c.member[q][1] >= 0) X[c.member[q][1]][i] = B.sub(E, O);
+                }
+            }
+        std::vector<std::vector<Ref>> Z(R);
+        for (int r = 0; r < R; r++) {
+            std::vector<Fr> hr(2 * m - 1, zero<FrParams>());
+            for (int D = 0; D < R; D++) {
+                if (is_zero(U[r][D])) continue;
+                for (int s = 0; s < 2 * m - 1; s++) hr[s] = add(hr[s], mul(U[r][D], h[D * m + s]));
+            }
+            Z[r] = hankel(B, X[r], hr);
+        }
+        std::vector<Ref> y(n);
+        for (int i = 0; i < m; i++) {
+            std::vector<std::vector<Ref>> W(cls.size(), std::vector<Ref>(6));
+            for (size_t ci = 0; ci < cls.size(); ci++) {
+                const Cls& c = cls[ci];
+                Ref S[3], D[3];
+                for (int q = 0; q < 3; q++) {
+                    const Ref zp = c.member[q][0] >= 0 ? Z[c.member[q][0]][i] : Ref{};
+                    const Ref zm = c.member[q][1] >= 0 ? Z[c.member[q][1]][i] : Ref{};
+                    S[q] = B.add(zp, zm);
+                    D[q] = B.sub(zp, zm);
+                }
+                for (int s = 0; s < 6 && s < k; s++) {
+                    const Ref* v = (s & 1) ? D : S;
+                    W[ci][s] = B.add(B.add(v[0], B.rotate(v[1], s)), B.rotate(v[2], 2 * s));
+                }
+            }
+            for (int I = 0; I < k; I++) {
+                std::vector<std::pair<Ref, int64_t>> t;
+                for (size_t ci = 0; ci < cls.size(); ci++) t.emplace_back(W[ci][I % 6], cf(cls[ci], I));
+                y[I * m + i] = sum(B, t);
+            }
+        }
+        return y;
+    }
+
     template <class SqrtFn>
     std::vector<Ref> twisted_cyclic(Builder& B, const std::vector<Ref>& x, const std::vector<Fr>& c, const Fr& z, SqrtFn&& sqrt_of) {
         const int n = (int)x.size();
@@ -347,10 +469,10 @@
         for (int n = 2; n <= max_n; n *= 2) {
             double best = 0;
             int best_k = 0;
-            for (int k : {2, 4, 8}) {
-                if (n % k || (k == 8 && !allow_toom8)) continue;
+            for (int k : {2, 4, 8, 16}) {
+                if (n % k || (k == 8 && !allow_toom8) || (k == 16 && !phi)) continue;
                 hankel_split[n] = k;
-                Builder B(n);
+                Builder B(n, lambda);
                 std::vector<Ref> x(n);
                 for (int i = 0; i < n; i++) x[i] = B.input(i);
                 std::vector<Fr> h(2 * n - 1);
@@ -362,7 +484,7 @@
             double cost[2];
             for (int split = 0; split < 2; split++) {
                 root_split[n] = split != 0;
-                Builder B(n);
+                Builder B(n, lambda);
                 std::vector<Ref> x(n);
                 for (int i = 0; i < n; i++) x[i] = B.input(i);
                 std::vector<Fr> c(n);
@@ -378,7 +500,7 @@
 private:
     const std::vector<std::vector<Fr>>& fixed_side(int k) {
         auto it = fixed_.find(k);
-        if (it == fixed_.end()) it = fixed_.emplace(k, toom_fixed_side(k)).first;
+        if (it == fixed_.end()) it = fixed_.emplace(k, toom_fixed_side(k, phi && k > 2, lambda)).first;
         return it->second;
     }
     std::map<int, std::vector<std::vector<Fr>>> fixed_;
@@ -387,10 +509,11 @@
 inline std::vector<Fr> run_over_fr(const Plan& p, const std::vector<Fr>& in) {
     std::vector<Fr> v(p.n_values, zero<FrParams>());
     for (int i = 0; i < p.n_in; i++) v[i] = in[i];
+    const Fr lp[3] = {one<FrParams>(), p.lambda, sqr(p.lambda)};
     for (auto& o : p.ops) {
         switch (o.kind) {
-            case OP_ADD: v[o.dst] = add(v[o.a], v[o.b]); break;
-            case OP_SUB: v[o.dst] = sub(v[o.a], v[o.b]); break;
+            case OP_ADD: v[o.dst] = add(v[o.a], mul(v[o.b], lp[o.rot])); break;
+            case OP_SUB: v[o.dst] = sub(v[o.a], mul(v[o.b], lp[o.rot])); break;
             case OP_DBL: { Fr t = v[o.a]; for (int k = 0; k < o.b; k++) t = add(t, t); v[o.dst] = t; break; }
             case OP_MULC: v[o.dst] = mul(v[o.a], p.consts[o.b]); break;
         }
@@ -398,7 +521,8 @@
     std::vector<Fr> out(p.outputs.size());
     for (size_t i = 0; i < out.size(); i++) {
         const Ref r = p.outputs[i];
-        out[i] = r.zero() ? zero<FrParams>() : (r.neg ? neg(v[r.id]) : v[r.id]);
+        const Fr t = r.zero() ? zero<FrParams>() : mul(v[r.id], lp[r.rot]);
+        out[i] = r.neg ? neg(t) : t;
     }
     return out;
 }
@@ -408,6 +532,8 @@
     std::map<int, int> hankel_split;
     std::map<int, bool> root_split;
     bool balanced_lincomb = false;
+    bool phi = true;
+    Fr lambda = glv_lambda();
 };
 inline Plan build_fk20_proofs_plan(const std::vector<Fr>& w128, const Strategy& strat, bool verbose = false) {
     if (w128.size() != 128) throw std::runtime_error("w128: need the 128 powers");
@@ -416,12 +542,16 @@
             if (eq(z, w128[e])) { s = w128[e / 2]; return true; }
         return false;
     };
+    if (strat.phi && !is_zero(add(add(sqr(strat.lambda), strat.lambda), one<FrParams>())))
+        throw std::runtime_error("fk20 plan: lambda is not a primitive cube root of unity");
     Compiler C;
     C.allow_toom8 = strat.allow_toom8;
     C.balanced_lincomb = strat.balanced_lincomb;
+    C.phi = strat.phi;
+    C.lambda = strat.lambda;
     if (strat.tuned) C.tune(32);
     else { C.hankel_split = strat.hankel_split; C.root_split = strat.root_split; }
-    Builder B(128);
+    Builder B(128, strat.lambda);
     const Fr one_ = one<FrParams>(), inv32 = inv(fr_small(32));
     auto m_of = [&](int e) {
         return mul(inv32, inv(sub(one_, w128[((e % 128) + 128) % 128])));
@@ -438,15 +568,15 @@
         out[2 * a + 1] = B.add(odd[a], t2[a]);
     }
     for (auto& r : out)
-        if (r.zero() || r.neg || r.id < 128) throw std::runtime_error("fk20 plan: degenerate output");
+        if (r.zero() || r.neg || r.rot || r.id < 128) throw std::runtime_error("fk20 plan: degenerate output");
     Plan p = B.take(out);
     if (verbose) {
         fprintf(stderr, "[linmap] hankel splits:");
         for (auto& kv : C.hankel_split) fprintf(stderr, " %d->%d", kv.first, kv.second);
         fprintf(stderr, "  root splits:");
         for (auto& kv : C.root_split) fprintf(stderr, " %d:%d", kv.first, (int)kv.second);
-        fprintf(stderr, "\n[linmap] %ld constant multiplications, %ld additions, %ld doublings\n", p.count(OP_MULC),
-                p.count(OP_ADD) + p.count(OP_SUB), p.doublings());
+        fprintf(stderr, "\n[linmap] %ld constant multiplications, %ld additions, %ld doublings, %ld phi operands, cost %.1f M\n",
+                p.count(OP_MULC), p.count(OP_ADD) + p.count(OP_SUB), p.doublings(), p.rotations(), Builder::plan_cost(p) / 1e6);
     }
     return p;
 }
@@ -483,6 +613,7 @@
     long mulc_total = 0;
     long fused_pairs = 0;
     long fused_runs = 0;
+    Fr lambda = glv_lambda();
 };
 inline Schedule make_schedule(const Plan& p, bool fuse_add_sub = true, bool fuse_runs = true) {
     const int n_out = (int)p.outputs.size();
@@ -518,7 +649,9 @@
             if (u.size() == 1 && two(u[0]) && fits(p.ops[u[0]])) ok = true;
             if (fuse_add_sub && u.size() == 2 && two(u[0]) && two(u[1]) && p.ops[u[0]].kind != p.ops[u[1]].kind) {
                 const Op &x = p.ops[u[0]], &y = p.ops[u[1]];
-                if (std::min(x.a, x.b) == std::min(y.a, y.b) && std::max(x.a, x.b) == std::max(y.a, y.b) && fits(x) && fits(y)) ok = true;
+                if (std::min(x.a, x.b) == std::min(y.a, y.b) && std::max(x.a, x.b) == std::max(y.a, y.b) && x.rot == y.rot &&
+                    (x.rot == 0 || x.a == y.a) && fits(x) && fits(y))
+                    ok = true;
             }
             if (!ok) continue;
             run_of[o.dst] = o.b;
@@ -569,6 +702,7 @@
         if (o.kind == OP_ADD || o.kind == OP_SUB) last_use[eff(o.b)] = std::max(last_use[eff(o.b)], s);
     }
     Schedule S;
+    S.lambda = p.lambda;
     std::vector<int> slot(p.n_values, -1);
     for (int i = 0; i < p.n_in; i++) slot[i] = i;
     for (int k = 0; k < n_out; k++) {
@@ -588,15 +722,18 @@
             else slot[v] = next_slot++;
         }
         for (int v : expire[s]) free_list.push_back(slot[v]);
-        std::map<std::pair<int, int>, int> add_of;
+        auto pair_key = [&](const Op& o) {
+            return o.rot ? std::make_tuple(o.a, o.b, o.rot) : std::make_tuple(std::min(o.a, o.b), std::max(o.a, o.b), 0);
+        };
+        std::map<std::tuple<int, int, int>, int> add_of;
         for (int i : step_ops[s])
-            if (p.ops[i].kind == OP_ADD) add_of[{std::min(p.ops[i].a, p.ops[i].b), std::max(p.ops[i].a, p.ops[i].b)}] = i;
+            if (p.ops[i].kind == OP_ADD) add_of[pair_key(p.ops[i])] = i;
         std::map<int, int> partner;
         std::vector<char> fused_away(p.ops.size(), 0);
         if (fuse_add_sub)
             for (int i : step_ops[s]) {
                 if (p.ops[i].kind != OP_SUB) continue;
-                auto it = add_of.find({std::min(p.ops[i].a, p.ops[i].b), std::max(p.ops[i].a, p.ops[i].b)});
+                auto it = add_of.find(pair_key(p.ops[i]));
                 if (it == add_of.end() || fused_away[it->second]) continue;
                 partner[i] = it->second;
                 fused_away[it->second] = 1;
@@ -616,9 +753,9 @@
                 const bool two = o.kind == OP_ADD || o.kind == OP_SUB;
                 if ((pass == 0) != (o.kind == OP_MULC)) continue;
                 if (fused_away[i]) continue;
-                int first = o.a, second = two ? o.b : 0;
-                if (two && run_of[o.b]) std::swap(first, second);
-                const uint32_t shifts = two ? (uint32_t)run_of[first] << 3 : 0u;
+                int first = o.a, second = two ? o.b : 0, rot_first = 0, rot_second = two ? o.rot : 0;
+                if (two && run_of[o.b]) { std::swap(first, second); std::swap(rot_first, rot_second); }
+                const uint32_t shifts = two ? ((uint32_t)run_of[first] << 3) | ((uint32_t)rot_first << 8) | ((uint32_t)rot_second << 10) : 0u;
                 if (two && run_of[first]) S.fused_runs++;
                 if (partner.count(i)) {
                     S.words.push_back((uint32_t)slot[p.ops[partner[i]].dst]);
@@ -646,6 +783,7 @@
 inline std::vector<Fr> run_schedule_over_fr(const Schedule& S, const std::vector<Fr>& consts, int n_in, int n_out, const std::vector<Fr>& in) {
     std::vector<Fr> arena(S.n_slots, zero<FrParams>());
     for (int i = 0; i < n_in; i++) arena[i] = in[i];
+    const Fr lp[4] = {one<FrParams>(), S.lambda, sqr(S.lambda), zero<FrParams>()};
     for (auto& L : S.launches) {
         std::vector<Fr> res(L.count), res2(L.count);
         for (int i = 0; i < L.count; i++) {
@@ -654,7 +792,7 @@
             if (L.kind == OP_MULC) res[i] = mul(a, consts[w[2]]);
             else if (w[3] & 2u) { Fr t = a; for (uint32_t k = 0; k < w[2]; k++) t = add(t, t); res[i] = t; }
             else {
-                Fr x = a, y = arena[w[2]];
+                Fr x = mul(a, lp[(w[3] >> 8) & 3u]), y = mul(arena[w[2]], lp[(w[3] >> 10) & 3u]);
                 for (uint32_t k = 0; k < ((w[3] >> 3) & 31u); k++) x = add(x, x);
                 if (w[3] & 4u) { res[i] = add(x, y); res2[i] = sub(x, y); }
                 else res[i] = (w[3] & 1u) ? sub(x, y) : add(x, y);
diff --git a/rust-eth-kzg_amd/csrc/k_g1slp.hip b/rust-eth-kzg_amd/csrc/k_g1slp.hip
--- a/rust-eth-kzg_amd/csrc/k_g1slp.hip
+++ b/rust-eth-kzg_amd/csrc/k_g1slp.hip
@@ -8,6 +8,16 @@
 
 static_assert(sizeof(JacS) == launch::SIZEOF_JACS && sizeof(JacQ) == launch::SIZEOF_JACQ, "the engine sizes and offsets the arena with these");
 
+__device__ __forceinline__ JacS slp_rotate(JacS p, uint32_t rot, const Fs<1, DC>& beta) {
+#pragma unroll 1
+    for (uint32_t k = 0; k < rot; k++) p = apply_phi(p, beta);
+    return p;
+}
+__device__ __forceinline__ JacQ slp_rotate(const JacQ& p, uint32_t rot, const Fs<1, DC>& beta) {
+    if (!rot) return p;
+    return jacq_from_jacs(slp_rotate(jacs_from_jacq(p), rot, beta));
+}
+
 __global__ __launch_bounds__(64, 2) void k_slp_mulc(JacQ* __restrict__ A, int stride, const uint32_t* __restrict__ words,
                                                     const uint32_t* __restrict__ naf, Fs<1, DC> beta, int n_active) {
     const uint32_t* w = words + (size_t)blockIdx.x * 4;
@@ -48,72 +58,75 @@
     const JacQ src = A[(size_t)a * stride + lane];
     A[(size_t)dst * stride + lane] = mul_by_recoded<2>(src, naf + (size_t)cid * (2 * launch::TWIDDLE_WORDS), beta, half);
 }
-__device__ __forceinline__ void slp_cheap_op(JacQ* __restrict__ A, int stride, int lane, uint32_t dst, uint32_t a, uint32_t b, uint32_t fl) {
-    JacQ r = A[(size_t)a * stride + lane];
+__device__ __forceinline__ void slp_cheap_op(JacQ* __restrict__ A, int stride, int lane, uint32_t dst, uint32_t a, uint32_t b, uint32_t fl,
+                                             const Fs<1, DC>& beta) {
+    const uint32_t rot_a = (fl & 2u) ? 0u : (fl >> 8) & 3u, rot_b = (fl & 2u) ? 0u : (fl >> 10) & 3u;
+    JacQ r = slp_rotate(A[(size_t)a * stride + lane], rot_a, beta);
     const uint32_t runs = (fl & 2u) ? b : (fl >> 3) & 31u;
 #pragma unroll 1
     for (uint32_t k = 0; k < runs; k++) r = dbl(r);
     bool degenerate = false;
     if (!(fl & 2u)) {
         if (fl & 4u) {
-            const AddSubShared sh = add_sub_prepare(r, A[(size_t)b * stride + lane]);
+            const AddSubShared sh = add_sub_prepare(r, slp_rotate(A[(size_t)b * stride + lane], rot_b, beta));
             degenerate = sh.degenerate;
             A[(size_t)(fl >> 16) * stride + lane] = add_sub_finish(sh, true);
             r = add_sub_finish(sh, false);
         } else {
-            r = add(r, A[(size_t)b * stride + lane], (fl & 1u) != 0);
+            r = add(r, slp_rotate(A[(size_t)b * stride + lane], rot_b, beta), (fl & 1u) != 0);
         }
     }
     A[(size_t)dst * stride + lane] = r;
     if (degenerate) {
         asm volatile("" ::: "memory");
-        JacQ p2 = A[(size_t)a * stride + lane];
+        JacQ p2 = slp_rotate(A[(size_t)a * stride + lane], rot_a, beta);
 #pragma unroll 1
         for (uint32_t k = 0; k < runs; k++) p2 = dbl(p2);
-        const JacQ q2 = A[(size_t)b * stride + lane];
+        const JacQ q2 = slp_rotate(A[(size_t)b * stride + lane], rot_b, beta);
         const JacQ d = add_slow(p2, q2, true);
         A[(size_t)dst * stride + lane] = add_slow(p2, q2, false);
         A[(size_t)(fl >> 16) * stride + lane] = d;
     }
 }
-__global__ __launch_bounds__(64, 2) void k_slp_add(JacQ* __restrict__ A, int stride, const uint32_t* __restrict__ words, int n_active) {
+__global__ __launch_bounds__(64, 2) void k_slp_add(JacQ* __restrict__ A, int stride, const uint32_t* __restrict__ words, Fs<1, DC> beta, int n_active) {
     const uint32_t* w = words + (size_t)blockIdx.y * 4;
     const uint32_t dst = __builtin_amdgcn_readfirstlane(w[0]), a = __builtin_amdgcn_readfirstlane(w[1]),
                    b = __builtin_amdgcn_readfirstlane(w[2]), fl = __builtin_amdgcn_readfirstlane(w[3]);
     if ((int)(blockIdx.x * 64 + threadIdx.x) >= n_active) return;
-    slp_cheap_op(A, stride, blockIdx.x * 64 + threadIdx.x, dst, a, b, fl);
-}
-
-__global__ __launch_bounds__(64, 2) void k_slp_add_s(JacS* __restrict__ A, int stride, const uint32_t* __restrict__ words, int n_active) {
+    slp_cheap_op(A, stride, blockIdx.x * 64 + threadIdx.x, dst, a, b, fl, beta);
+}
+
+__global__ __launch_bounds__(64, 2) void k_slp_add_s(JacS* __restrict__ A, int stride, const uint32_t* __restrict__ words, Fs<1, DC> beta, int n_active) {
     const uint32_t* w = words + (size_t)blockIdx.y * 4;
     const uint32_t dst = __builtin_amdgcn_readfirstlane(w[0]), a = __builtin_amdgcn_readfirstlane(w[1]),
                    b = __builtin_amdgcn_readfirstlane(w[2]), fl = __builtin_amdgcn_readfirstlane(w[3]);
     const int lane_of_thread = blockIdx.x * 64 + threadIdx.x;
     const bool keep = lane_of_thread < n_active;
     const int lane = keep ? lane_of_thread : n_active - 1;
-    JacS r = A[(size_t)a * stride + lane];
+    const uint32_t rot_a = (fl & 2u) ? 0u : (fl >> 8) & 3u, rot_b = (fl & 2u) ? 0u : (fl >> 10) & 3u;
+    JacS r = slp_rotate(A[(size_t)a * stride + lane], rot_a, beta);
     const uint32_t runs = (fl & 2u) ? b : (fl >> 3) & 31u;
 #pragma unroll 1
     for (uint32_t k = 0; k < runs; k++) r = dbl_half(r);
     bool degenerate = false;
     if (!(fl & 2u)) {
         if (fl & 4u) {
-            const AddSubSharedS sh = add_sub_prepare(r, A[(size_t)b * stride + lane]);
+            const AddSubSharedS sh = add_sub_prepare(r, slp_rotate(A[(size_t)b * stride + lane], rot_b, beta));
             degenerate = sh.degenerate;
             const JacS df = add_sub_finish(sh, true);
             if (keep) A[(size_t)(fl >> 16) * stride + lane] = df;
             r = add_sub_finish(sh, false);
         } else {
-            r = add_unchecked(r, A[(size_t)b * stride + lane], (fl & 1u) != 0, degenerate);
+            r = add_unchecked(r, slp_rotate(A[(size_t)b * stride + lane], rot_b, beta), (fl & 1u) != 0, degenerate);
         }
     }
     if (keep) A[(size_t)dst * stride + lane] = r;
     if (degenerate && keep) {
         asm volatile("" ::: "memory");
-        JacS p2 = A[(size_t)a * stride + lane];
+        JacS p2 = slp_rotate(A[(size_t)a * stride + lane], rot_a, beta);
 #pragma unroll 1
         for (uint32_t k = 0; k < runs; k++) p2 = dbl_half(p2);
-        const JacS q2 = A[(size_t)b * stride + lane];
+        const JacS q2 = slp_rotate(A[(size_t)b * stride + lane], rot_b, beta);
         if (fl & 4u) {
             const JacS d = add_slow(p2, q2, true);
             A[(size_t)dst * stride + lane] = add_slow(p2, q2, false);
@@ -124,18 +137,19 @@
     }
 }
 
-__global__ __launch_bounds__(64, 2) void k_slp_add_coop(JacQ* __restrict__ A, int stride, const uint32_t* __restrict__ words, int lanes) {
+__global__ __launch_bounds__(64, 2) void k_slp_add_coop(JacQ* __restrict__ A, int stride, const uint32_t* __restrict__ words, Fs<1, DC> beta, int lanes) {
     const uint32_t* w = words + (size_t)blockIdx.y * 4;
     const uint32_t dst = __builtin_amdgcn_readfirstlane(w[0]), a = __builtin_amdgcn_readfirstlane(w[1]),
                    b = __builtin_amdgcn_readfirstlane(w[2]), fl = __builtin_amdgcn_readfirstlane(w[3]);
     const int lane = blockIdx.x * 16 + (threadIdx.x >> 2), quad = threadIdx.x & 3;
     if (lane >= lanes) return;
-    JacQ r = A[(size_t)a * stride + lane];
+    const uint32_t rot_a = (fl & 2u) ? 0u : (fl >> 8) & 3u, rot_b = (fl & 2u) ? 0u : (fl >> 10) & 3u;
+    JacQ r = slp_rotate(A[(size_t)a * stride + lane], rot_a, beta);
     const uint32_t runs = (fl & 2u) ? b : (fl >> 3) & 31u;
 #pragma unroll 1
     for (uint32_t k = 0; k < runs; k++) r = coop_dbl(r, quad);
     if (!(fl & 2u)) {
-        const JacQ q = A[(size_t)b * stride + lane];
+        const JacQ q = slp_rotate(A[(size_t)b * stride + lane], rot_b, beta);
         if (fl & 4u) {
             const JacQ d = coop_add(r, q, true, quad);
             A[(size_t)(fl >> 16) * stride + lane] = d;
@@ -160,19 +174,20 @@
     const JacS r = mul_by_recoded30<COOP>(src, naf + (size_t)cid * (2 * launch::TWIDDLE_WORDS), beta, sub);
     if (keep) A[(size_t)dst * stride + lane] = r;
 }
-__global__ __launch_bounds__(64, 2) void k_slp_add_coop_s(JacS* __restrict__ A, int stride, const uint32_t* __restrict__ words, int lanes) {
+__global__ __launch_bounds__(64, 2) void k_slp_add_coop_s(JacS* __restrict__ A, int stride, const uint32_t* __restrict__ words, Fs<1, DC> beta, int lanes) {
     const uint32_t* w = words + (size_t)blockIdx.y * 4;
     const uint32_t dst = __builtin_amdgcn_readfirstlane(w[0]), a = __builtin_amdgcn_readfirstlane(w[1]),
                    b = __builtin_amdgcn_readfirstlane(w[2]), fl = __builtin_amdgcn_readfirstlane(w[3]);
     const int lane_of_thread = blockIdx.x * 16 + (threadIdx.x >> 2), quad = threadIdx.x & 3;
     const bool keep = lane_of_thread < lanes;
     const int lane = keep ? lane_of_thread : lanes - 1;
-    JacS r = A[(size_t)a * stride + lane];
+    const uint32_t rot_a = (fl & 2u) ? 0u : (fl >> 8) & 3u, rot_b = (fl & 2u) ? 0u : (fl >> 10) & 3u;
+    JacS r = slp_rotate(A[(size_t)a * stride + lane], rot_a, beta);
     const uint32_t runs = (fl & 2u) ? b : (fl >> 3) & 31u;
 #pragma unroll 1
     for (uint32_t k = 0; k < runs; k++) r = coop4_dbl_half(r, quad);
     if (!(fl & 2u)) {
-        const JacS q = A[(size_t)b * stride + lane];
+        const JacS q = slp_rotate(A[(size_t)b * stride + lane], rot_b, beta);
         if (fl & 4u) {
             JacS d;
             coop4_add_sub(r, q, quad, r, d);
@@ -194,12 +209,12 @@
     if (lanes <= 0) lanes = stride;
     if (n_active <= 0 || n_active > lanes) n_active = lanes;
     const dim3 grid((unsigned)count, (unsigned)(lanes / 64));
+    Fp b384;
+    for (int i = 0; i < 12; i++) b384.v[i] = beta.v[i];
+    const Fs<1, DC> bs = fs_from_fp(b384);
     if (fmt == FMT_JACS) {
         const bool coop = coop_points_max() > 0;
         if (kind == 3) {
-            Fp b384;
-            for (int i = 0; i < 12; i++) b384.v[i] = beta.v[i];
-            const Fs<1, DC> bs = fs_from_fp(b384);
             if (coop_lanes > 16 && coop)
                 k_slp_mulc_coop_s<2><<<dim3((unsigned)count, (unsigned)((coop_lanes + 31) / 32)), 64, 0, st>>>((JacS*)arena, stride, words, (const uint32_t*)naf, bs, coop_lanes);
             else if (coop_lanes > 0 && coop)
@@ -207,14 +222,12 @@
             else k_slp_mulc_s<<<grid, 64, 0, st>>>((JacS*)arena, stride, words, (const uint32_t*)naf, bs, n_active);
         } else {
             if (lanes == 64 && count * 4 <= 1024 && coop)
-                k_slp_add_coop_s<<<dim3((unsigned)((n_active + 15) / 16), (unsigned)count), 64, 0, st>>>((JacS*)arena, stride, words, n_active);
-            else k_slp_add_s<<<dim3((unsigned)(lanes / 64), (unsigned)count), 64, 0, st>>>((JacS*)arena, stride, words, n_active);
+                k_slp_add_coop_s<<<dim3((unsigned)((n_active + 15) / 16), (unsigned)count), 64, 0, st>>>((JacS*)arena, stride, words, bs, n_active);
+            else k_slp_add_s<<<dim3((unsigned)(lanes / 64), (unsigned)count), 64, 0, st>>>((JacS*)arena, stride, words, bs, n_active);
         }
         return;
     }
     if (kind == 3) {
-        Fp b384;
-        for (int i = 0; i < 12; i++) b384.v[i] = beta.v[i];
         if (coop_lanes > 16 && coop_points_max() > 0) {
             const dim3 g2((unsigned)count, (unsigned)((coop_lanes + 31) / 32));
             k_slp_mulc_coop2<<<g2, 64, 0, st>>>((JacQ*)arena, stride, words, (const uint32_t*)naf, fq_from_fp(b384), coop_lanes);
@@ -222,12 +235,12 @@
         else if (coop_lanes > 0 && coop_points_max() > 0)
             k_slp_mulc_coop<<<dim3((unsigned)count, (unsigned)((coop_lanes + 15) / 16)), 64, 0, st>>>((JacQ*)arena, stride, words, (const uint32_t*)naf,
                                                                                                      fq_from_fp(b384), coop_lanes);
-        else k_slp_mulc<<<grid, 64, 0, st>>>((JacQ*)arena, stride, words, (const uint32_t*)naf, fs_from_fp(b384), n_active);
+        else k_slp_mulc<<<grid, 64, 0, st>>>((JacQ*)arena, stride, words, (const uint32_t*)naf, bs, n_active);
     } else {
         if (lanes == 64 && count * 4 <= 1024 && coop_points_max() > 0)
-            k_slp_add_coop<<<dim3((unsigned)((n_active + 15) / 16), (unsigned)count), 64, 0, st>>>((JacQ*)arena, stride, words, n_active);
-        else k_slp_add<<<dim3((unsigned)(lanes / 64), (unsigned)count), 64, 0, st>>>((JacQ*)arena, stride, words, n_active);
-    }
-}
-}
-}
+            k_slp_add_coop<<<dim3((unsigned)((n_active + 15) / 16), (unsigned)count), 64, 0, st>>>((JacQ*)arena, stride, words, bs, n_active);
+        else k_slp_add<<<dim3((unsigned)(lanes / 64), (unsigned)count), 64, 0, st>>>((JacQ*)arena, stride, words, bs, n_active);
+    }
+}
+}
+}
```

New measurement: 41120, median of 6. 1.02x the previous value.
